# jh-jeong/ContraD

Hardware: AMD Instinct MI355X
Metric: discriminator-step images/sec (ContraD, SimCLR aug) (higher is better)
Workload: dtype f32; 1 GPU; SNDCGAN + ContraD D-step, CIFAR-10 32x32, global batch 512, simclr aug, nonsat loss, Adam(2e-4,(0.5,0.999)), random-init weights; global_batch=512, per_gpu_batch=512, parallelism=dp1, losses_finite=True, launch=hipGraph replay, rccl_ranks=1

## Files before the change

### contrad_amd/csrc/igemm.hip

```cpp
#include "common.h"
#include <stdlib.h>
#include <string.h>
#include <algorithm>
#include <utility>
#include "../../include/contrad_hip.h"

namespace {

enum { MODE_FWD = 0, MODE_DGRAD = 1, MODE_WGRAD = 2 };
#ifndef IGEMM_BK
#define IGEMM_BK 16
#endif
constexpr int BK = IGEMM_BK;
#ifndef IGEMM_MIN_WAVES
#define IGEMM_MIN_WAVES 4
#endif
constexpr int NTHREADS = 256;

struct IgemmArgs {
  const float* A;
  const float* B;
  float* C;
  const float* bias;
  const float* addend;
  const float* act_ref;
  float* bias_ws;
  contrad_conv_desc d;
  float slope, gain;
  int M, Ncol, Kg;
  int tiles_m, tiles_n;
  int P;
  int ptiles_per_split;
  int ny;
  int cgroup;
  int cbal;
  int cb_reps[4], cb_start[5];
  int dsplits;
  long long slab_elems;
  int px_pixels;
  short win_h0[16], win_w0[16], win_hc[16], win_wc[16];
  int win_tile0[17];
  int nwin;
  unsigned char px_order[256];
  int pixmajor;
  int px_full;
  int st_nt;
};

constexpr long long NT_STORE_BYTES = 256ll << 20;
inline int st_nt_for(long long rows, int ld) {
#if defined(LEAN_ST_NT)
  if (LEAN_ST_NT >= 0) return LEAN_ST_NT;
#endif
  return rows * (long long)ld * (long long)sizeof(float) >= NT_STORE_BYTES ? 1 : 0;
}

__device__ __forceinline__ float4 ld4(const float* p) { return *reinterpret_cast<const float4*>(p); }
__device__ __forceinline__ float4 zero4() { return make_float4(0.f, 0.f, 0.f, 0.f); }

template <int MODE, int BM, int BN, bool VEC>
__global__ __launch_bounds__(NTHREADS, 2) void igemm_kernel(const IgemmArgs p) {
  extern __shared__ __attribute__((aligned(16))) float smem[];
  constexpr bool A_KCONTIG = (MODE != MODE_WGRAD);
  constexpr bool B_KCONTIG = (MODE == MODE_DGRAD);
  constexpr int LDA = BM + (A_KCONTIG ? 1 : 4);
  constexpr int LDB = BN + (B_KCONTIG ? 1 : 4);
  constexpr int A_SZ = BK * LDA, B_SZ = BK * LDB;
  constexpr int PA = BM * BK / 1024, PB = BN * BK / 1024;
  constexpr int KQ = BK / 4;
  constexpr int KROWS = NTHREADS / KQ;
  constexpr int WM = BM / 2, WN = BN / 2, TM = WM / 32, TN = WN / 32;
  constexpr int EPV = VEC ? 1 : 4;

  const contrad_conv_desc& d = p.d;
  const int tid = threadIdx.x;
  const int lane = tid & 63, wave = tid >> 6;
  const int wm = wave >> 1, wn = wave & 1;

  const int b = xcd_remap(blockIdx.x, gridDim.x);
  const int tile_n = b % p.tiles_n, tile_m = b / p.tiles_n;
  const int m0 = tile_m * BM, n0 = tile_n * BN;

  int M = p.M, Ncol = p.Ncol, Kg = p.Kg;
  int ph = 0, pw = 0, Hc = 0, Wc = 0, kh0 = 0, kw0 = 0, nth = 0, ntw = 1, bh = 0, bw = 0;
  if constexpr (MODE == MODE_DGRAD) {
    const int s = d.stride;
    ph = blockIdx.y / s;
    pw = blockIdx.y % s;
    Hc = (d.H - ph + s - 1) / s;
    Wc = (d.W - pw + s - 1) / s;
    kh0 = (ph + d.pad) % s;
    kw0 = (pw + d.pad) % s;
    nth = (kh0 < d.KH) ? (d.KH - kh0 + s - 1) / s : 0;
    ntw = (kw0 < d.KW) ? (d.KW - kw0 + s - 1) / s : 0;
    bh = (ph + d.pad - kh0) / s;
    bw = (pw + d.pad - kw0) / s;
    M = d.N * Hc * Wc;
    Ncol = d.C;
    Kg = nth * ntw * d.K;
    if (ntw == 0) ntw = 1;
    if (m0 >= M) return;
  }
  int p_begin = 0, p_end = 0;
  if constexpr (MODE == MODE_WGRAD) {
    p_begin = blockIdx.y * p.ptiles_per_split * BK;
    p_end = min(p.P, p_begin + p.ptiles_per_split * BK);
  }
  const int T = (MODE == MODE_WGRAD) ? ((p_end > p_begin) ? (p_end - p_begin + BK - 1) / BK : 0)
                                     : (Kg + BK - 1) / BK;

  const int kq = tid % KQ, krow = tid / KQ;
  constexpr int A_RPP = 1024 / BM, B_RPP = 1024 / BN;
  const int a_c4 = tid % (BM / 4), a_r = tid / (BM / 4);
  const int b_c4 = tid % (BN / 4), b_r = tid / (BN / 4);

  int a_n[PA], a_h[PA], a_w[PA];
  bool a_ok[PA];
  int wg_dn = 0, wg_dh = 0, wg_dw = 0;
  int wg_pbase = 0;

  if constexpr (MODE == MODE_FWD) {
#pragma unroll
    for (int i = 0; i < PA; ++i) {
      const int m = m0 + krow + KROWS * i;
      a_ok[i] = m < M;
      const int mm = a_ok[i] ? m : 0;
      const int wo = mm % d.Wo, t = mm / d.Wo;
      const int ho = t % d.Ho;
      a_n[i] = t / d.Ho;
      a_h[i] = ho * d.stride - d.pad;
      a_w[i] = wo * d.stride - d.pad;
    }
  } else if constexpr (MODE == MODE_DGRAD) {
#pragma unroll
    for (int i = 0; i < PA; ++i) {
      const int m = m0 + krow + KROWS * i;
      a_ok[i] = m < M;
      const int mm = a_ok[i] ? m : 0;
      const int wq = mm % Wc, t = mm / Wc;
      a_n[i] = t / Hc;
      a_h[i] = t % Hc + bh;
      a_w[i] = wq + bw;
    }
  } else {
    const int hw = d.Ho * d.Wo;
    wg_pbase = p_begin;
    wg_dn = BK / hw;
    const int rem = BK - wg_dn * hw;
    wg_dh = rem / d.Wo;
    wg_dw = rem - wg_dh * d.Wo;
#pragma unroll
    for (int i = 0; i < PA; ++i) {
      const int pp = p_begin + a_r + A_RPP * i;
      const int wo = pp % d.Wo, t = pp / d.Wo;
      a_w[i] = wo;
      a_h[i] = t % d.Ho;
      a_n[i] = t / d.Ho;
      a_ok[i] = true;
    }
  }

  float4 ra[PA], rb[PB];
  unsigned amask = 0, bmask = 0;

  auto fwd_a = [&](int i, int k, bool& ok) -> size_t {
    const int kk = (k < Kg) ? k : 0;
    const int tap = kk / d.C, c = kk - tap * d.C;
    const int kh = tap / d.KW, kw = tap - kh * d.KW;
    const int hi = a_h[i] + kh, wi = a_w[i] + kw;
    ok = (k < Kg) && a_ok[i] && (unsigned)hi < (unsigned)d.H && (unsigned)wi < (unsigned)d.W;
    return ok ? ((size_t)(a_n[i] * d.H + hi) * d.W + wi) * d.ldx + c : 0;
  };
  auto dg_decode = [&](int k, int& th, int& tw, int& co, int& tapflat) {
    const int kk = (k < Kg) ? k : 0;
    const int ti = kk / d.K;
    co = kk - ti * d.K;
    th = ti / ntw;
    tw = ti - th * ntw;
    tapflat = (kh0 + d.stride * th) * d.KW + (kw0 + d.stride * tw);
  };
  auto wg_a = [&](int i, int ic, bool pok, bool& ok) -> size_t {
    const int icc = (ic < Kg) ? ic : 0;
    const int tap = icc / d.C, c = icc - tap * d.C;
    const int kh = tap / d.KW, kw = tap - kh * d.KW;
    const int hi = a_h[i] * d.stride - d.pad + kh, wi = a_w[i] * d.stride - d.pad + kw;
    ok = pok && (ic < Kg) && (unsigned)hi < (unsigned)d.H && (unsigned)wi < (unsigned)d.W;
    return ok ? ((size_t)(a_n[i] * d.H + hi) * d.W + wi) * d.ldx + c : 0;
  };

  auto load_a_generic = [&](int t) {
    const int k0 = t * BK;
    amask = 0;
    if constexpr (MODE == MODE_FWD) {
      const int k = k0 + kq * 4;
#pragma unroll
      for (int i = 0; i < PA; ++i) {
        if constexpr (VEC) {
          bool ok;
          const size_t off = fwd_a(i, k, ok);
          ra[i] = ld4(p.A + off);
// ... 2028 lines not shown
  if (contrad_conv2d_path(d, mode) != 3) return 1.0;
  return mode == MODE_DGRAD ? dgrad_valid_tap_fraction(d) : fwd_valid_tap_fraction(d);
}

extern "C" long long contrad_conv2d_grid_blocks(const contrad_conv_desc* d, int mode, int with_workspace) {
  if (check_desc(d) || mode < 0 || mode > 2) return -22;
  if (mode != MODE_WGRAD && with_workspace && wino44_planned(d, mode)) return wino44_grid(wino44_args(d, mode));
  if (mode != MODE_WGRAD && with_workspace && wino_planned(d, mode)) return wino_grid(wino_args(d, mode));
  if (with_workspace && wino23_planned(d, mode)) return wino23_grid(wino23_args(d));
  if (mode != MODE_WGRAD && with_workspace && wino22_planned(d, mode)) {
    const wino22::Args a = wino22_args(d, mode);
    return 8 * std::min(WINO_CUS / 8, cdiv(a.NTB, 8) * a.NKB * (mode == MODE_DGRAD ? 4 : 1));
  }
  if (mode == MODE_FWD) {
    const FwdPlan p = fwd_plan(d);
    const long long M = (long long)d->N * d->Ho * d->Wo;
    if (fwd_k1_ok(d)) return cdivll(M, 4);
    if (conv_c32_ok(d)) return conv_c32_blocks(d);
    if (p.pixmajor == 1) return (long long)cdiv(d->N, p.bm) * d->Ho * d->Wo * cdiv(d->K, p.bn);
    if (p.pixmajor == 2) return (long long)border_class_tiles(d, MODE_FWD, p.bm) * cdiv(d->K, p.bn);
    return cdivll(M, p.bm) * cdiv(d->K, p.bn) * (with_workspace ? p.splits : 1);
  }
  if (mode == MODE_DGRAD) {
    if (conv_c32_ok(d)) return conv_c32_blocks(d);
    const int s = d->stride;
    const long long Mc = (long long)d->N * cdiv(d->H, s) * cdiv(d->W, s);
    const FwdPlan p = dgrad_plan(d, with_workspace != 0);
    const int tiles_m = p.pixmajor == 2 ? border_class_tiles(d, MODE_DGRAD, p.bm)
                        : p.pixmajor == 1 ? cdiv(d->N, p.bm) * cdiv(d->H, s) * cdiv(d->W, s) : cdiv((int)Mc, p.bm);
    const int tiles_n = cdiv(d->C, p.bn);
    if (p.splits > 1) return (long long)tiles_m * tiles_n * p.splits;
    if (p.balanced && vec_ok(d, MODE_DGRAD) && lean_ok(d, MODE_DGRAD, 0) && p.pixmajor == 0) {
      IgemmArgs a{};
      const long long blocks = dgrad_balance(d, tiles_m, &a);
      if (blocks > 0) return blocks * tiles_n;
    }
    if (p.pixmajor == 1 && s == 2) return (long long)tiles_m * tiles_n * s * s;
    const int cgroup = (s > 1) ? dgrad_cgroup(tiles_m, tiles_n) : 0;
    const int tm_pad = cgroup > 0 ? cdiv(tiles_m, cgroup) * cgroup : tiles_m;
    return (long long)tm_pad * tiles_n * s * s;
  }
  if (wino_wgrad_planned(d)) { const wino::WArgs a = wino_wgrad_args(d); return (long long)a.CB * a.KB * wino_wgrad_splits(a); }
  if (wino22_wgrad_planned(d)) { const wino22::WArgs a = wino22_wgrad_args(d); return (long long)a.RBN * a.KB * wino22_wgrad_splits(a); }
  if (wgrad_c32_ok(d)) return wgrad_c32_blocks(d);
  int bm, bn, tm, tn, splits, pps;
  wgrad_plan(d, &bm, &bn, &tm, &tn, &splits, &pps);
  return (long long)tm * tn * splits;
}

extern "C" int contrad_conv2d_tile_order(const contrad_conv_desc* d, int mode, unsigned char* out, int capacity) {
  if (check_desc(d) || (mode != MODE_FWD && mode != MODE_DGRAD) || !out || capacity <= 0) return -22;
  int taps[256];
  unsigned char full[256];
  int nt = 0;
  if (mode == MODE_FWD) {
    const FwdPlan p = fwd_plan(d);
    if (p.pixmajor != 1 || !vec_ok(d, MODE_FWD)) return 0;
    for (int ho = 0; ho < d->Ho; ++ho)
      for (int wo = 0; wo < d->Wo; ++wo) {
        int vh = 0, vw = 0;
        for (int kh = 0; kh < d->KH; ++kh) vh += (unsigned)(ho * d->stride - d->pad + kh) < (unsigned)d->H;
        for (int kw = 0; kw < d->KW; ++kw) vw += (unsigned)(wo * d->stride - d->pad + kw) < (unsigned)d->W;
        taps[ho * d->Wo + wo] = vh * vw;
      }
    if (!pixel_order_full(taps, d->Ho * d->Wo, cdiv(d->N, p.bm), cdiv(d->K, p.bn), full, 8)) return 0;
    nt = cdiv(d->N, p.bm) * d->Ho * d->Wo;
  } else {
    const FwdPlan p = dgrad_plan(d, true);
    if (p.pixmajor != 1 || p.splits > 1 || !vec_ok(d, MODE_DGRAD)) return 0;
    if (d->stride == 1) {
      for (int h = 0; h < d->H; ++h)
        for (int w = 0; w < d->W; ++w) {
          int vh = 0, vw = 0;
          for (int kh = 0; kh < d->KH; ++kh) vh += (unsigned)(h + d->pad - kh) < (unsigned)d->Ho;
          for (int kw = 0; kw < d->KW; ++kw) vw += (unsigned)(w + d->pad - kw) < (unsigned)d->Wo;
          taps[h * d->W + w] = vh * vw;
        }
      if (!pixel_order_full(taps, d->H * d->W, cdiv(d->N, p.bm), cdiv(d->C, p.bn), full, 8)) return 0;
      nt = cdiv(d->N, p.bm) * d->H * d->W;
    } else {
      const int npix = dgrad_strided_class0_taps(d, taps);
      if (!npix || !dgrad_strided_full_ok(d, p.bm, p.bn)) return 0;
      pixel_order_full(taps, npix, cdiv(d->N, p.bm), cdiv(d->C, p.bn), full, 2);
      nt = cdiv(d->N, p.bm) * npix;
    }
  }
  if (nt > capacity) return -22;
  memcpy(out, full, (size_t)nt);
  return nt;
}

extern "C" long long contrad_conv2d_wgrad_workspace_bytes(const contrad_conv_desc* d) {
  if (check_desc(d)) return -22;
  if (wino_wgrad_planned(d)) return wino_wgrad_workspace_bytes(d);
  if (wino22_wgrad_planned(d)) return wino22_wgrad_workspace_bytes(d);
  if (wgrad_c32_ok(d))
    return (long long)wgrad_c32_blocks(d) * ((long long)d->KH * d->KW * d->C + 1) * d->K * (long long)sizeof(float);
  int bm, bn, tm, tn, splits, pps;
  wgrad_plan(d, &bm, &bn, &tm, &tn, &splits, &pps);
  return (long long)splits * ((long long)d->KH * d->KW * d->C + 1) * d->K * (long long)sizeof(float);
}

extern "C" int contrad_conv2d_wgrad(const contrad_conv_desc* d, const float* x, const float* gy,
                                    float* dwp, float* dbias, float* workspace, long long workspace_bytes,
                                    contrad_stream_t stream) {
  int rc = check_desc(d);
  if (rc) return rc;
  CONTRAD_ARG(x && gy && dwp && workspace);
  if (vec_ok(d, MODE_WGRAD)) CONTRAD_ARG(aligned16(x, gy, workspace));
  CONTRAD_ARG(workspace_bytes >= contrad_conv2d_wgrad_workspace_bytes(d));
  if (wino_wgrad_planned(d)) return launch_wino_wgrad(d, x, gy, dwp, dbias, workspace, (hipStream_t)stream);
  if (wino22_wgrad_planned(d)) return launch_wino22_wgrad(d, x, gy, dwp, dbias, workspace, (hipStream_t)stream);
  if (wgrad_c32_ok(d)) {
    const int blocks = wgrad_c32_blocks(d);
    const long long total = (long long)d->KH * d->KW * d->C * d->K;
    float* bias_ws = dbias ? workspace + (size_t)blocks * total : nullptr;
    rc = launch_wgrad_c32(d, x, gy, workspace, bias_ws, (hipStream_t)stream);
    if (rc) return rc;
    int R = 1;
    while (R < 64 && R * 2 <= blocks && (total / 4) * R < 65536) R <<= 1;
    long long rb = ((total / 4) * R + 255) / 256;
    if (rb > 2048) rb = 2048;
    hipLaunchKernelGGL(wgrad_reduce_kernel, dim3((int)rb), dim3(256), 0, (hipStream_t)stream, workspace, dwp,
                       d->KH * d->KW * d->C, d->K, d->ldw, blocks, bias_ws, dbias, R);
    CONTRAD_CHECK_LAUNCH();
    return 0;
  }
  int bm, bn, splits, pps;
  IgemmArgs a{};
  wgrad_plan(d, &bm, &bn, &a.tiles_m, &a.tiles_n, &splits, &pps);
  a.A = x; a.B = gy; a.C = workspace; a.d = *d;
  a.M = d->KH * d->KW * d->C; a.Ncol = d->K; a.Kg = a.M;
  const bool fused_bias = dbias != nullptr && vec_ok(d, MODE_WGRAD);
  CONTRAD_ARG(dbias == nullptr || fused_bias);
  a.bias_ws = fused_bias ? workspace + (size_t)splits * a.M * a.Ncol : nullptr;
  const long long P = (long long)d->N * d->Ho * d->Wo;
  CONTRAD_ARG(P < (1ll << 31) - 4096);
  a.P = (int)P; a.ptiles_per_split = pps;
  a.pixmajor = wgrad_pixmajor_ok(d, bm, pps) ? 1 : 0;
  rc = dispatch<MODE_WGRAD>(a, bm, bn, vec_ok(d, MODE_WGRAD), dim3(a.tiles_m * a.tiles_n, splits),
                            (hipStream_t)stream);
  if (rc) return rc;
  const long long total = (long long)a.M * a.Ncol;
  int R = 1;
  while (R < 64 && R * 2 <= splits && (total / 4) * R < 65536) R <<= 1;
  long long blocks = ((total / 4) * R + 255) / 256;
  if (blocks > 2048) blocks = 2048;
  if (blocks < 1) blocks = 1;
  hipLaunchKernelGGL(wgrad_reduce_kernel, dim3((int)blocks), dim3(256), 0, (hipStream_t)stream, workspace, dwp,
                     a.M, a.Ncol, d->ldw, splits, a.bias_ws, fused_bias ? dbias : nullptr, R);
  CONTRAD_CHECK_LAUNCH();
  return 0;
}
```

### contrad_amd/csrc/igemm_lean.h

```cpp
#pragma once

#ifndef LEAN_DEEP
#define LEAN_DEEP 0
#endif
#ifndef LEAN_LD_NT
#define LEAN_LD_NT 0
#endif
#ifndef LEAN_ST_NT
#define LEAN_ST_NT -1
#endif
#ifndef LEAN_QPAD
#define LEAN_QPAD 8
#endif

constexpr unsigned LEAN_OOB = 0x80000000u;
constexpr unsigned LEAN_RANGE = 0x80000000u;
constexpr unsigned WB_TOP = 2u, WB_BOT = 4u, WB_LEFT = 8u, WB_RIGHT = 16u;

__device__ __forceinline__ float4 bload4(__amdgpu_buffer_rsrc_t r, unsigned voff, unsigned soff) {
  return __builtin_bit_cast(float4, __builtin_amdgcn_raw_buffer_load_b128(r, (int)voff, (int)soff, 0));
}

__device__ __forceinline__ __amdgpu_buffer_rsrc_t lean_rsrc(const float* base, bool on) {
  return __builtin_amdgcn_make_buffer_rsrc(const_cast<float*>(base), 0, on ? (int)LEAN_RANGE : 0, 0x00020000);
}

template <class P> struct lean_par_value { static constexpr int v = 0; };
template <int V> struct lean_par_value<std::integral_constant<int, V>> { static constexpr int v = V; };

__device__ __forceinline__ int pow2_shift(int d) { return (d & (d - 1)) == 0 ? __builtin_ctz(d) : -1; }
__device__ __forceinline__ void divmod_u(int x, int d, int sh, int& q, int& r) {
  if (sh >= 0) { q = x >> sh; r = x & (d - 1); }
  else { q = x / d; r = x - q * d; }
}

template <int MODE, int BM, int BN, bool BAL>
__device__ __forceinline__ void lean_tile(const IgemmArgs& p, float* smem, const int tile_m, const int tile_n, const int by,
                                          const int wc_h0, const int wc_w0, const int wc_hc, const int wc_wc) {
  static_assert(BK == 16, "the lean loop is written for a 16-deep K-tile");
  static_assert(!BAL || MODE == MODE_DGRAD, "balanced order: strided data gradient only");
  const int pl_pixmajor = BAL ? 0 : p.pixmajor, pl_nwin = BAL ? 0 : p.nwin, pl_dsplits = BAL ? 0 : p.dsplits;
  constexpr bool A_Q = (MODE != MODE_WGRAD);
  constexpr bool B_Q = (MODE == MODE_DGRAD);
  constexpr int QSA = BM * 4 + LEAN_QPAD, QSB = BN * 4 + LEAN_QPAD;
  constexpr int LDB = BN < 64 ? 64 : BN;
  constexpr int A_SZ = A_Q ? 4 * QSA : 16 * BM;
  constexpr int B_SZ = B_Q ? 4 * QSB : 16 * LDB;
  constexpr int BUF = A_SZ + B_SZ;
  constexpr int PA = BM / 64, PB = BN < 64 ? 1 : BN / 64;
  constexpr int A_RPP = 1024 / BM, B_RPP = 1024 / BN;
  constexpr bool B_HALF = BN < 64;
  constexpr int WAVES_N = BN < 64 ? 1 : 2, WAVES_M = 4 / WAVES_N;
  constexpr int WM = BM / WAVES_M, WN = BN / WAVES_N, TM = WM / 32, TN = WN / 32;
  static_assert(TM >= 1 && TN >= 1, "tile too small for the wave arrangement");

  const contrad_conv_desc& d = p.d;
  const int tid = threadIdx.x;
  const int lane = tid & 63, wave = tid >> 6;
  const int wm = wave / WAVES_N, wn = wave % WAVES_N;
  const int l31 = lane & 31, lhi = lane >> 5;

  const int m0 = tile_m * BM, n0 = tile_n * BN;

  const int kq = tid & 3, qrow = tid >> 2;
  const int a_c4 = tid % (BM / 4), a_r = tid / (BM / 4);
  const int b_c4 = tid % (BN / 4), b_r = tid / (BN / 4);

  int M = p.M, Ncol = p.Ncol;
  int T = 0;
  unsigned tapmask = 0xFFFFFFFFu;
  unsigned wskip = 0;
  long long px_off = 0;
  int px_pitch = 0, px_rows = 0;
  const float* baseA = p.A;
  const float* baseB = p.B;
  unsigned va[PA], vb[PB];
  unsigned inv[PA];

  int u_tap = 0, u_a = 0, u_b = 0, u_c0 = 0;
  int u_n = 0, u_h = 0, u_w = 0;
  int ph = 0, pw = 0, Hc = 0, Wc = 0, kh0 = 0, kw0 = 0, nth = 0, ntw = 1, bh = 0, bw = 0;
  int gw = 1, gh = 1, gn = 1, n_begin = 0;

  if constexpr (MODE == MODE_FWD) {
    const int t_total = p.Kg / BK, t_begin = by * p.ptiles_per_split;
    T = min(p.ptiles_per_split, t_total - t_begin);
    if (T < 0) T = 0;
    const int ntaps = d.KH * d.KW;
    u_c0 = (t_begin / ntaps) * BK;
    u_tap = t_begin % ntaps;
    u_a = u_tap / d.KW;
    u_b = u_tap - u_a * d.KW;
    const int HoWo = d.Ho * d.Wo;
    if (pl_pixmajor) {
      int ib, pix;
      if (p.px_full) {
        const int e = p.px_order[tile_m];
        ib = e / HoWo; pix = e - ib * HoWo;
      } else {
        ib = tile_m / HoWo; pix = p.px_order[tile_m - ib * HoWo];
      }
      const int ho = pix / d.Wo, wo = pix - ho * d.Wo;
      const int n_first = ib * BM;
      unsigned wmask = 0, valid = 0;
      for (int kw = 0; kw < d.KW; ++kw) wmask |= ((unsigned)(wo * d.stride - d.pad + kw) < (unsigned)d.W ? 1u : 0u) << kw;
      for (int kh = 0; kh < d.KH; ++kh)
        if ((unsigned)(ho * d.stride - d.pad + kh) < (unsigned)d.H) valid |= wmask << (kh * d.KW);
      tapmask = valid ? valid : 0xFFFFFFFFu;
      T = __builtin_popcount(valid) * (d.C / BK);
      u_tap = valid ? __builtin_ctz(valid) : 0;
      u_a = u_tap / d.KW;
      u_b = u_tap - u_a * d.KW;
      u_c0 = 0;
      baseA = p.A + ((long long)n_first * d.H * d.W + (long long)(ho * d.stride - d.pad) * d.W + (wo * d.stride - d.pad)) * d.ldx;
      const int img = d.H * d.W * d.ldx;
#pragma unroll
      for (int i = 0; i < PA; ++i) {
        const int r = qrow + 64 * i;
        va[i] = (unsigned)((r * img + kq * 4) * 4);
        inv[i] = (n_first + r < d.N) ? 0u : 0xFFFFFFFFu;
      }
      px_off = ((long long)n_first * HoWo + pix) * d.ldy;
      px_pitch = HoWo * d.ldy;
      px_rows = min(BM, d.N - n_first);
    }
    const bool win = pl_nwin > 0;
    const int gHo = win ? wc_hc : d.Ho, gWo = win ? wc_wc : d.Wo;
    if (win) {
      M = d.N * gHo * gWo;
      unsigned wmask = 0, valid = 0;
      for (int kw = 0; kw < d.KW; ++kw) wmask |= ((unsigned)(wc_w0 * d.stride - d.pad + kw) < (unsigned)d.W ? 1u : 0u) << kw;
      for (int kh = 0; kh < d.KH; ++kh)
        if ((unsigned)(wc_h0 * d.stride - d.pad + kh) < (unsigned)d.H) valid |= wmask << (kh * d.KW);
      tapmask = valid ? valid : 0xFFFFFFFFu;
      T = __builtin_popcount(valid) * (d.C / BK);
      u_tap = valid ? __builtin_ctz(valid) : 0;
      u_a = u_tap / d.KW;
      u_b = u_tap - u_a * d.KW;
      u_c0 = 0;
      if (m0 >= M) return;
    }
    const int sh_w = pow2_shift(gWo), sh_h = pow2_shift(gHo);
    const int n_first = (sh_w >= 0 && sh_h >= 0) ? (m0 >> (sh_w + sh_h)) : m0 / (gHo * gWo);
    if (!pl_pixmajor) baseA = p.A + ((long long)n_first * d.H * d.W - (d.pad * d.W + d.pad)) * d.ldx;
#pragma unroll
    for (int i = 0; i < PA; ++i) {
      if (pl_pixmajor) break;
      const int m = m0 + qrow + 64 * i;
      const bool ok = m < M;
      const int mm = ok ? m : m0;
      int wo, t, ho, n;
      divmod_u(mm, gWo, sh_w, t, wo);
      divmod_u(t, gHo, sh_h, n, ho);
      ho += wc_h0; wo += wc_w0;
      va[i] = (unsigned)(((((n - n_first) * d.H + ho * d.stride) * d.W + wo * d.stride) * d.ldx + kq * 4) * 4);
      unsigned wmask = 0, valid = 0;
      for (int kw = 0; kw < d.KW; ++kw) wmask |= ((unsigned)(wo * d.stride - d.pad + kw) < (unsigned)d.W ? 1u : 0u) << kw;
      for (int kh = 0; kh < d.KH; ++kh)
        if ((unsigned)(ho * d.stride - d.pad + kh) < (unsigned)d.H) valid |= wmask << (kh * d.KW);
      inv[i] = ok ? ~valid : 0xFFFFFFFFu;
    }
#pragma unroll
    for (int i = 0; i < PB; ++i) {
      const int col = n0 + b_c4 * 4;
      vb[i] = (col < Ncol && b_r + B_RPP * i < BK) ? (unsigned)((((b_r + B_RPP * i) * d.ldw) + col) * 4) : LEAN_OOB;
    }
  } else if constexpr (MODE == MODE_DGRAD) {
    const int s = d.stride;
    const int cls = (pl_dsplits > 1) ? 0 : by;
    ph = cls / s;
    pw = cls % s;
    Hc = (d.H - ph + s - 1) / s;
    Wc = (d.W - pw + s - 1) / s;
    kh0 = (ph + d.pad) % s;
    kw0 = (pw + d.pad) % s;
    nth = (kh0 < d.KH) ? (d.KH - kh0 + s - 1) / s : 0;
    ntw = (kw0 < d.KW) ? (d.KW - kw0 + s - 1) / s : 0;
    bh = (ph + d.pad - kh0) / s;
    bw = (pw + d.pad - kw0) / s;
    M = d.N * Hc * Wc;
    Ncol = d.C;
    T = nth * ntw * d.K / BK;
    if (pl_dsplits > 1) {
      const int t_begin = by * p.ptiles_per_split, ntaps = nth * ntw;
      T = min(p.ptiles_per_split, T - t_begin);
      if (T < 0) T = 0;
      u_c0 = (t_begin / ntaps) * BK;
      u_tap = t_begin % ntaps;
      u_a = u_tap / ntw;
      u_b = u_tap - u_a * ntw;
    }
    if (ntw == 0) ntw = 1;
    if (pl_nwin > 0) {
      Hc = wc_hc; Wc = wc_wc;
      M = d.N * Hc * Wc;
      const int ah0 = wc_h0 + bh, aw0 = wc_w0 + bw;
      unsigned wmask = 0, valid = 0;
      for (int tw = 0; tw < ntw; ++tw) wmask |= ((unsigned)(aw0 - tw) < (unsigned)d.Wo ? 1u : 0u) << tw;
      for (int th = 0; th < nth; ++th)
        if ((unsigned)(ah0 - th) < (unsigned)d.Ho) valid |= wmask << (th * ntw);
      tapmask = valid ? valid : 0xFFFFFFFFu;
      T = __builtin_popcount(valid) * (d.K / BK);
      u_tap = valid ? __builtin_ctz(valid) : 0;
      u_a = u_tap / ntw;
      u_b = u_tap - u_a * ntw;
      u_c0 = 0;
    }
    const int HcWc = Hc * Wc;
    if (pl_pixmajor) {
      int ib, cpix;
      if (p.px_full) {
        const int e = p.px_order[tile_m];
        ib = e / p.px_pixels; cpix = e - ib * p.px_pixels;
      } else {
        ib = tile_m / p.px_pixels; cpix = p.px_order[tile_m - ib * p.px_pixels];
      }
      if (cpix >= HcWc) return;
      int hq = cpix / Wc, wq = cpix - hq * Wc;
      if (p.px_full == 2) {
        if (ph) hq = Hc - 1 - hq;
        if (pw) wq = Wc - 1 - wq;
      }
      const int ah = hq + bh, aw = wq + bw;
      const int n_first = ib * BM;
      unsigned wmask = 0, valid = 0;
      for (int tw = 0; tw < ntw; ++tw) wmask |= ((unsigned)(aw - tw) < (unsigned)d.Wo ? 1u : 0u) << tw;
      for (int th = 0; th < nth; ++th)
        if ((unsigned)(ah - th) < (unsigned)d.Ho) valid |= wmask << (th * ntw);
      tapmask = valid ? valid : 0xFFFFFFFFu;
      T = __builtin_popcount(valid) * (d.K / BK);
      u_tap = valid ? __builtin_ctz(valid) : 0;
      u_a = u_tap / ntw;
      u_b = u_tap - u_a * ntw;
      u_c0 = 0;
      M = d.N;
      baseA = p.A + ((long long)n_first * d.Ho * d.Wo + (long long)(ah - (nth - 1)) * d.Wo + (aw - (ntw - 1))) * d.ldy;
      const int img = d.Ho * d.Wo * d.ldy;
#pragma unroll
      for (int i = 0; i < PA; ++i) {
        const int r = qrow + 64 * i;
        va[i] = (unsigned)((r * img + kq * 4) * 4);
        inv[i] = (n_first + r < d.N) ? 0u : 0xFFFFFFFFu;
      }
      px_off = ((long long)n_first * d.H * d.W + (long long)(hq * s + ph) * d.W + (wq * s + pw)) * d.ldx;
      px_pitch = d.H * d.W * d.ldx;
      px_rows = min(BM, d.N - n_first);
    }
    if (!pl_pixmajor && m0 >= M) return;
    const int sh_w = pow2_shift(Wc), sh_h = pow2_shift(Hc);
    const int n_first = (sh_w >= 0 && sh_h >= 0) ? (m0 >> (sh_w + sh_h)) : m0 / HcWc;
    if (!pl_pixmajor) baseA = p.A + ((long long)n_first * d.Ho * d.Wo - ((nth - 1) * d.Wo + (ntw - 1))) * d.ldy;
#pragma unroll
    for (int i = 0; i < PA; ++i) {
      if (pl_pixmajor) break;
      const int m = m0 + qrow + 64 * i;
      const bool ok = m < M;
      const int mm = ok ? m : m0;
      int wq, t, n, hq;
      divmod_u(mm, Wc, sh_w, t, wq);
      divmod_u(t, Hc, sh_h, n, hq);
      hq += wc_h0; wq += wc_w0;
      const int ah = hq + bh, aw = wq + bw;
      va[i] = (unsigned)(((((n - n_first) * d.Ho + ah) * d.Wo + aw) * d.ldy + kq * 4) * 4);
      unsigned wmask = 0, valid = 0;
      for (int tw = 0; tw < ntw; ++tw) wmask |= ((unsigned)(aw - tw) < (unsigned)d.Wo ? 1u : 0u) << tw;
      for (int th = 0; th < nth; ++th)
        if ((unsigned)(ah - th) < (unsigned)d.Ho) valid |= wmask << (th * ntw);
      inv[i] = ok ? ~valid : 0xFFFFFFFFu;
    }
#pragma unroll
    for (int i = 0; i < PB; ++i) {
      const int c = n0 + qrow + 64 * i;
      vb[i] = (c < Ncol && qrow + 64 * i < BN) ? (unsigned)((c * d.ldw + kq * 4) * 4) : LEAN_OOB;
    }
  } else {
    const int tiles_total = p.P / BK;
    const int t_begin = by * p.ptiles_per_split;
    T = min(p.ptiles_per_split, tiles_total - t_begin);
    if (T < 0) T = 0;
    gw = min(d.Wo, 16);
    gh = min(d.Ho, 16 / gw);
    if (pl_pixmajor) { gw = 1; gh = 1; }
    gn = 16 / (gw * gh);
    const int tpr = d.Wo / gw, tpi = tpr * (d.Ho / gh);
    u_w = (t_begin % tpr) * gw;
    u_h = ((t_begin / tpr) % (d.Ho / gh)) * gh;
    u_n = (t_begin / tpi) * gn;
    n_begin = u_n;
    baseA = p.A + ((long long)n_begin * d.H * d.W - (d.pad * d.W + d.pad)) * d.ldx;
    baseB = pl_pixmajor ? p.B + (long long)n_begin * d.Ho * d.Wo * d.ldy : p.B + (long long)t_begin * BK * d.ldy;
    if (pl_pixmajor) {
      const int tap0 = m0 / d.C;
      const int kh = tap0 / d.KW, kw = tap0 - kh * d.KW;
      const int chh = kh - d.pad, cww = kw - d.pad;
      const int hb = (d.Ho - 1) * d.stride, wb = (d.Wo - 1) * d.stride;
      wskip = ((unsigned)chh < (unsigned)d.H ? 0u : WB_TOP) | ((unsigned)(hb + chh) < (unsigned)d.H ? 0u : WB_BOT) |
              ((unsigned)cww < (unsigned)d.W ? 0u : WB_LEFT) | ((unsigned)(wb + cww) < (unsigned)d.W ? 0u : WB_RIGHT);
      if (p.bias_ws != nullptr && tile_m == 0) wskip = 0;
      int hh = u_h, ww = u_w, cnt = 0, first = -1;
      for (int q = 0; q < T; ++q) {
        const unsigned e = (hh == 0 ? WB_TOP : 0u) | (hh == d.Ho - 1 ? WB_BOT : 0u) | (ww == 0 ? WB_LEFT : 0u) | (ww == d.Wo - 1 ? WB_RIGHT : 0u);
        if (!(wskip & e)) { ++cnt; if (first < 0) first = q; }
        if (++ww == d.Wo) { ww = 0; if (++hh == d.Ho) hh = 0; }
      }
      T = cnt;
      if (cnt == 0) wskip = 0;
      for (int q = 0; q < first; ++q) {
        u_w += 1;
        if (u_w == d.Wo) { u_w = 0; u_h += 1; if (u_h == d.Ho) { u_h = 0; u_n += gn; } }
      }
    }
    const int ic = m0 + a_c4 * 4;
    const bool colok = ic < p.Kg;
    const int icc = colok ? ic : 0;
    const int tap = icc / d.C, c = icc - tap * d.C;
    const int kh = tap / d.KW, kw = tap - kh * d.KW;
#pragma unroll
    for (int i = 0; i < PA; ++i) {
      const int r = a_r + A_RPP * i;
      const int dw = r % gw, dh = (r / gw) % gh, dn = r / (gw * gh);
      const int chh = dh * d.stride - d.pad + kh, cww = dw * d.stride - d.pad + kw;
      const int hb = (d.Ho - gh) * d.stride, wb = (d.Wo - gw) * d.stride;
      inv[i] = ((unsigned)chh < (unsigned)d.H ? 0u : WB_TOP) | ((unsigned)(hb + chh) < (unsigned)d.H ? 0u : WB_BOT) |
               ((unsigned)cww < (unsigned)d.W ? 0u : WB_LEFT) | ((unsigned)(wb + cww) < (unsigned)d.W ? 0u : WB_RIGHT);
      va[i] = colok ? (unsigned)((((dn * d.H + dh * d.stride + kh) * d.W + dw * d.stride + kw) * d.ldx + c) * 4)
                    : LEAN_OOB;
    }
#pragma unroll
    for (int i = 0; i < PB; ++i) {
      const int col = n0 + b_c4 * 4;
      const int rowpitch = pl_pixmajor ? d.Ho * d.Wo * d.ldy : d.ldy;
      vb[i] = (col < Ncol && b_r + B_RPP * i < BK) ? (unsigned)((((b_r + B_RPP * i) * rowpitch) + col) * 4) : LEAN_OOB;
    }
  }

  constexpr bool DEEP = ((LEAN_DEEP & 1) && MODE == MODE_WGRAD && BM * BN <= 128 * 64) ||
                        ((LEAN_DEEP & 2) && MODE != MODE_WGRAD && BM * BN <= 128 * 64);
  constexpr int NSET = DEEP ? 2 : 1;
  float4 ra[NSET][PA], rb[NSET][PB];
  unsigned soffA = 0, soffB = 0;
  unsigned edge = 0;
  auto wgrad_pos_edge = [&]() -> unsigned {
    return (u_h == 0 ? WB_TOP : 0u) | (u_h == d.Ho - gh ? WB_BOT : 0u) | (u_w == 0 ? WB_LEFT : 0u) | (u_w == d.Wo - gw ? WB_RIGHT : 0u);
  };
  unsigned pos_edge = (MODE == MODE_WGRAD) ? wgrad_pos_edge() : 0u;
  unsigned pos_offA = 0, pos_offB = 0, wk_aw = 0, wk_ah = 0, wk_an = 0, wk_b = 0, wk_bh = 0, wk_bn = 0;
  (void)wk_bh;
  if constexpr (MODE == MODE_FWD) {
    pos_offA = (unsigned)(((u_a * d.W + u_b) * d.ldx + u_c0) * 4);
    pos_offB = (unsigned)((u_tap * d.C + u_c0) * d.ldw * 4);
    wk_aw = (unsigned)(d.ldx * 4);
    wk_ah = (unsigned)((d.W - d.KW) * d.ldx * 4);
    wk_an = (unsigned)((BK - d.KH * d.W * d.ldx) * 4);
    wk_b = (unsigned)(d.C * d.ldw * 4);
    wk_bn = (unsigned)((BK - d.KH * d.KW * d.C) * d.ldw * 4);
  } else if constexpr (MODE == MODE_DGRAD) {
    pos_offA = (unsigned)((((nth - 1 - u_a) * d.Wo + (ntw - 1 - u_b)) * d.ldy + u_c0) * 4);
    pos_offB = (unsigned)((((kh0 + d.stride * u_a) * d.KW + (kw0 + d.stride * u_b)) * d.C * d.ldw + u_c0) * 4);
    wk_aw = (unsigned)(-d.ldy * 4);
    wk_ah = (unsigned)((ntw - d.Wo) * d.ldy * 4);
    wk_an = (unsigned)((nth * d.Wo * d.ldy + BK) * 4);
    wk_b = (unsigned)(d.stride * d.C * d.ldw * 4);
    wk_bh = (unsigned)(d.stride * (d.KW - ntw) * d.C * d.ldw * 4);
    wk_bn = (unsigned)((BK - d.stride * nth * d.KW * d.C * d.ldw) * 4);
  }
  if constexpr (MODE == MODE_WGRAD) {
    pos_offA = (unsigned)(((((u_n - n_begin) * d.H + u_h * d.stride) * d.W + u_w * d.stride) * d.ldx) * 4);
    pos_offB = pl_pixmajor ? (unsigned)((((u_n - n_begin) * d.Ho + u_h) * d.Wo + u_w) * d.ldy * 4) : 0u;
    wk_aw = (unsigned)(gw * d.stride * d.ldx * 4);
    wk_ah = (unsigned)((gh * d.stride * d.W - d.Wo * d.stride) * d.ldx * 4);
    wk_an = (unsigned)((gn * d.H - d.Ho * d.stride) * d.W * d.ldx * 4);
    wk_b = (unsigned)((pl_pixmajor ? 1 : BK) * d.ldy * 4);
    wk_bn = pl_pixmajor ? (unsigned)((gn - 1) * d.Ho * d.Wo * d.ldy * 4) : 0u;
  }
  int t_next = 0;
  __amdgpu_buffer_rsrc_t rsA = lean_rsrc(baseA, false), rsB = lean_rsrc(baseB, false);

  auto begin_tile = [&]() {
    const bool on = t_next < T;
    rsA = lean_rsrc(baseA, on);
    rsB = lean_rsrc(baseB, on);
    soffA = pos_offA;
    soffB = pos_offB;
    if constexpr (MODE == MODE_WGRAD) edge = pos_edge;
  };
  auto end_tile = [&]() {
    ++t_next;
    if constexpr (MODE == MODE_FWD) {
      do {
        ++u_tap; ++u_b; pos_offA += wk_aw; pos_offB += wk_b;
        if (u_b == d.KW) {
          u_b = 0; ++u_a; pos_offA += wk_ah;
          if (u_a == d.KH) { u_a = 0; u_tap = 0; pos_offA += wk_an; pos_offB += wk_bn; }
        }
      } while (!((tapmask >> u_tap) & 1u));
    } else if constexpr (MODE == MODE_DGRAD) {
      do {
        ++u_tap; ++u_b; pos_offA += wk_aw; pos_offB += wk_b;
        if (u_b == ntw) {
          u_b = 0; ++u_a; pos_offA += wk_ah; pos_offB += wk_bh;
          if (u_a == nth) { u_a = 0; u_tap = 0; pos_offA += wk_an; pos_offB += wk_bn; }
        }
      } while (!((tapmask >> u_tap) & 1u));
    } else {
      do {
        u_w += gw; pos_offA += wk_aw; pos_offB += wk_b;
        if (u_w == d.Wo) {
          u_w = 0; u_h += gh; pos_offA += wk_ah;
          if (u_h == d.Ho) { u_h = 0; u_n += gn; pos_offA += wk_an; pos_offB += wk_bn; }
        }
        pos_edge = wgrad_pos_edge();
      } while (wskip & pos_edge);
    }
  };
  auto load_a_piece = [&](int set, int i) {
    unsigned v;
    if constexpr (MODE == MODE_WGRAD) {
      v = (inv[i] & edge) ? LEAN_OOB : va[i];
    } else {
      v = va[i] | ((inv[i] >> u_tap) << 31);
    }
    ra[set][i] = bload4(rsA, v, soffA);
  };
  auto load_b_piece = [&](int set, int i) { rb[set][i] = bload4(rsB, vb[i], soffB); };

  int wrA, wrB, rdA[TM], rdB[TN];
  if constexpr (A_Q) {
    wrA = kq * QSA + qrow * 4;
#pragma unroll
    for (int i = 0; i < TM; ++i) rdA[i] = lhi * QSA + (wm * WM + i * 32 + l31) * 4;
  } else {
    wrA = a_r * BM + ((a_c4 * 4) ^ (((a_r >> 2) & 1) * 32));
#pragma unroll
    for (int i = 0; i < TM; ++i) rdA[i] = 4 * lhi * BM + ((wm * WM + i * 32 + l31) ^ (32 * lhi));
  }
  if constexpr (B_Q) {
    wrB = A_SZ + kq * QSB + qrow * 4;
#pragma unroll
    for (int j = 0; j < TN; ++j) rdB[j] = A_SZ + lhi * QSB + (wn * WN + j * 32 + l31) * 4;
  } else {
    wrB = A_SZ + b_r * LDB + ((b_c4 * 4) ^ (((b_r >> 2) & 1) * 32));
#pragma unroll
    for (int j = 0; j < TN; ++j) rdB[j] = A_SZ + 4 * lhi * LDB + ((wn * WN + j * 32 + l31) ^ (32 * lhi));
  }

  float4 colacc = zero4();
  const bool do_bias = (MODE == MODE_WGRAD) && p.bias_ws != nullptr && tile_m == 0;

  auto store_a_piece = [&](int bufoff, int set, int i) {
    float* dst = smem + bufoff + wrA + (A_Q ? i * 256 : i * A_RPP * BM);
    *reinterpret_cast<float4*>(dst) = ra[set][i];
  };
  const bool b_owner = !B_HALF || (B_Q ? qrow < BN : b_r < BK);
  auto store_b_piece = [&](int bufoff, int set, int i) {
    float* dst = smem + bufoff + wrB + (B_Q ? i * 256 : i * B_RPP * LDB);
    if (b_owner) *reinterpret_cast<float4*>(dst) = rb[set][i];
    if constexpr (MODE == MODE_WGRAD) {
      if (do_bias) {
        asm volatile("" ::: "memory");
        colacc.x += rb[set][i].x; colacc.y += rb[set][i].y; colacc.z += rb[set][i].z; colacc.w += rb[set][i].w;
      }
    }
  };

  f32x16 acc[TM][TN];
#pragma unroll
  for (int i = 0; i < TM; ++i)
#pragma unroll
    for (int j = 0; j < TN; ++j)
#pragma unroll
      for (int r = 0; r < 16; ++r) acc[i][j][r] = 0.f;

  if (T > 0) {
    begin_tile();
#pragma unroll
    for (int i = 0; i < PA; ++i) load_a_piece(0, i);
#pragma unroll
    for (int i = 0; i < PB; ++i) load_b_piece(0, i);
    end_tile();
    if constexpr (DEEP) {
      begin_tile();
#pragma unroll
      for (int i = 0; i < PA; ++i) load_a_piece(1, i);
#pragma unroll
      for (int i = 0; i < PB; ++i) load_b_piece(1, i);
      end_tile();
    }
#pragma unroll
    for (int i = 0; i < PA; ++i) store_a_piece(0, 0, i);
#pragma unroll
    for (int i = 0; i < PB; ++i) store_b_piece(0, 0, i);
  }
  __syncthreads();

  constexpr bool RAGGED_SKIP = (MODE == MODE_WGRAD) && BN <= 64;
  const bool wave_on = !RAGGED_SKIP || __builtin_amdgcn_readfirstlane((m0 + wm * WM < M) ? 1 : 0) != 0;

  constexpr int KS = BK / 2;
#ifndef IGEMM_ST_SHIFT
#define IGEMM_ST_SHIFT 1
#endif
  constexpr int A_LD0 = 0, B_LD0 = PA, A_ST0 = KS - PA - PB - IGEMM_ST_SHIFT, B_ST0 = KS - PB - IGEMM_ST_SHIFT;
  static_assert(A_ST0 >= A_LD0 + PA - 1 && B_ST0 >= B_LD0 + PB - 1 && A_ST0 >= 0,
                "a piece must be stored after its own load was issued");
  constexpr bool UNROLL2 = !(BM * BN > 128 * 64 && MODE != MODE_WGRAD);
  static_assert(!DEEP || UNROLL2, "the two-deep prefetch needs the buffer parity at compile time");
  auto k_tile = [&](auto par, auto with_mfma, const int t) {
    const int cur = (int)par * BUF, nxt = BUF - cur;
    (void)t;
    float fa[2][TM][4], fb[2][TN][4];
#if defined(LEAN_ABLATE_FRAGS)
#pragma unroll
    for (int h = 0; h < 2; ++h)
#pragma unroll
      for (int j = 0; j < 4; ++j) {
#pragma unroll
        for (int i = 0; i < TM; ++i) fa[h][i][j] = (float)(t + i + j);
#pragma unroll
        for (int i = 0; i < TN; ++i) fb[h][i][j] = (float)(t - i - j);
      }
#else
#pragma unroll
    for (int h = 0; h < 2; ++h) {
#pragma unroll
      for (int i = 0; i < TM; ++i) {
        if constexpr (A_Q) {
          const float4 q = *reinterpret_cast<const float4*>(smem + cur + rdA[i] + 2 * h * QSA);
          fa[h][i][0] = q.x; fa[h][i][1] = q.y; fa[h][i][2] = q.z; fa[h][i][3] = q.w;
        } else {
#pragma unroll
          for (int j = 0; j < 4; ++j) fa[h][i][j] = smem[cur + rdA[i] + (8 * h + j) * BM];
        }
      }
#pragma unroll
      for (int i = 0; i < TN; ++i) {
        if constexpr (B_Q) {
          const float4 q = *reinterpret_cast<const float4*>(smem + cur + rdB[i] + 2 * h * QSB);
          fb[h][i][0] = q.x; fb[h][i][1] = q.y; fb[h][i][2] = q.z; fb[h][i][3] = q.w;
        } else {
#pragma unroll
          for (int j = 0; j < 4; ++j) fb[h][i][j] = smem[cur + rdB[i] + (8 * h + j) * LDB];
        }
      }
    }
#endif
    __builtin_amdgcn_sched_barrier(0);
#pragma unroll
    for (int ks = 0; ks < KS; ++ks) {
      const int h = ks >> 2, j = ks & 3;
#if !defined(LEAN_ABLATE_LOADS)
      constexpr int LSET = DEEP ? lean_par_value<decltype(par)>::v : 0, SSET = DEEP ? 1 - lean_par_value<decltype(par)>::v : 0;
      if (ks == A_LD0) begin_tile();
      if (ks >= A_LD0 && ks < A_LD0 + PA) load_a_piece(LSET, ks - A_LD0);
      if (ks >= B_LD0 && ks < B_LD0 + PB) load_b_piece(LSET, ks - B_LD0);
      if (ks == B_LD0 + PB - 1) end_tile();
#endif
      __builtin_amdgcn_sched_barrier(0);
      if constexpr (decltype(with_mfma)::value) {
#pragma unroll
        for (int i = 0; i < TM; ++i)
#pragma unroll
          for (int jj = 0; jj < TN; ++jj)
            acc[i][jj] = __builtin_amdgcn_mfma_f32_32x32x2f32(fa[h][i][j], fb[h][jj][j], acc[i][jj], 0, 0, 0);
      }
      __builtin_amdgcn_sched_barrier(0);
// ... 114 lines not shown
          }
        }
      }
    };
    if (st_nt && !(MODE == MODE_DGRAD && pl_dsplits > 1)) store_rows(std::true_type{}); else store_rows(std::false_type{});
  } else {
    const bool slab = (MODE == MODE_WGRAD) || p.ny > 1;
    const bool pxm = (MODE == MODE_FWD) && pl_pixmajor;
    const int pitch = pxm ? px_pitch : (slab ? Ncol : d.ldy);
    const size_t out_off = pxm ? (size_t)px_off : (slab ? (size_t)by * M * Ncol : (size_t)0) + (size_t)m0 * pitch;
    float* outp = p.C + out_off;
    const int rows_here = pxm ? px_rows : min(BM, M - m0);
    const __amdgpu_buffer_rsrc_t rsC = __builtin_amdgcn_make_buffer_rsrc(outp, 0, rows_here * pitch * 4, 0x00020000);
    const int wave_row = __builtin_amdgcn_readfirstlane(wm * WM);
    const float g1 = p.gain, g0 = p.gain * p.slope;
    const bool has_add = (MODE == MODE_FWD) && !slab && p.addend != nullptr;
    const __amdgpu_buffer_rsrc_t rsD = __builtin_amdgcn_make_buffer_rsrc(
        const_cast<float*>(has_add ? p.addend + out_off : outp), 0, has_add ? rows_here * pitch * 4 : 0, 0x00020000);
    unsigned lanepart[TN];
    float bj[TN];
#pragma unroll
    for (int j = 0; j < TN; ++j) {
      lanepart[j] = colpart[j] + (unsigned)(4 * lhi * pitch) * 4u;
      const int c = n0 + wn * WN + j * 32 + l31;
      bj[j] = (MODE == MODE_FWD && !slab && p.bias && c < Ncol) ? p.bias[c] : 0.f;
    }
    if constexpr (MODE == MODE_FWD) {
      constexpr int EPI_F = (BM * BN > 128 * 64) ? 4 : EPI_G;
      auto store_fwd = [&](auto nt_c) {
      constexpr int ST_AUX = decltype(nt_c)::value ? 2 : 0;
      constexpr int LD_AUX = (LEAN_LD_NT && decltype(nt_c)::value) ? 2 : 0;
#pragma unroll
      for (int i = 0; i < TM; ++i)
#pragma unroll
        for (int r0 = 0; r0 < 16; r0 += EPI_F) {
          unsigned rowpart[EPI_F];
#pragma unroll
          for (int q = 0; q < EPI_F; ++q) {
            const int r = r0 + q;
            rowpart[q] = (unsigned)((wave_row + i * 32 + (r & 3) + 8 * (r >> 2)) * pitch) * 4u;
          }
          float rv[EPI_F][TN];
          if (has_add) {
#pragma unroll
            for (int q = 0; q < EPI_F; ++q)
#pragma unroll
              for (int j = 0; j < TN; ++j)
                rv[q][j] = __builtin_bit_cast(float, __builtin_amdgcn_raw_buffer_load_b32(rsD, (int)(lanepart[j] + rowpart[q]), 0, LD_AUX));
          }
#pragma unroll
          for (int q = 0; q < EPI_F; ++q)
#pragma unroll
            for (int j = 0; j < TN; ++j) {
              float v = acc[i][j][r0 + q];
              if (!slab) {
                v += bj[j];
                v *= (v > 0.f) ? g1 : g0;
                if (has_add) v += rv[q][j];
              }
              __builtin_amdgcn_raw_buffer_store_b32(__builtin_bit_cast(unsigned, v), rsC, (int)(lanepart[j] + rowpart[q]), 0, ST_AUX);
            }
        }
      };
      if (st_nt && !slab) store_fwd(std::true_type{}); else store_fwd(std::false_type{});
    } else {
#pragma unroll
      for (int i = 0; i < TM; ++i)
#pragma unroll
        for (int r = 0; r < 16; ++r) {
          const unsigned rowpart = (unsigned)((wave_row + i * 32 + (r & 3) + 8 * (r >> 2)) * pitch) * 4u;
#pragma unroll
          for (int j = 0; j < TN; ++j) {
            const float v = acc[i][j][r];
            __builtin_amdgcn_raw_buffer_store_b32(__builtin_bit_cast(unsigned, v), rsC, (int)(lanepart[j] + rowpart), 0, 0);
          }
        }
    }
    if constexpr (MODE == MODE_WGRAD) {
      if (do_bias) {
        float* red = smem;
        *reinterpret_cast<float4*>(red + b_r * BN + b_c4 * 4) = colacc;
        __syncthreads();
        if (tid < BN) {
          float sum = 0.f;
#pragma unroll
          for (int r = 0; r < B_RPP; ++r) sum += red[r * BN + tid];
          const int c = n0 + tid;
          if (c < Ncol) p.bias_ws[(size_t)by * Ncol + c] = sum;
        }
      }
    }
  }
}

template <int MODE, int BM, int BN, bool BAL = false>
__global__ __launch_bounds__(NTHREADS, IGEMM_MIN_WAVES) void igemm_lean_kernel(const IgemmArgs p) {
  extern __shared__ __attribute__((aligned(16))) float smem[];
  const int lin = xcd_remap(blockIdx.x, gridDim.x);
  int by, tile_n, tile_m;
  int nrep = 1;
  int wc_h0 = 0, wc_w0 = 0, wc_hc = 0, wc_wc = 0;
  if constexpr (MODE == MODE_WGRAD) {
    const int tiles = p.tiles_m * p.tiles_n;
    by = lin / tiles;
    const int b = lin - by * tiles;
    tile_n = b % p.tiles_n; tile_m = b / p.tiles_n;
  } else if constexpr (BAL) {
    const int per_group = p.cb_start[4] * p.tiles_n;
    const int g = lin / per_group, r = lin - g * per_group;
    const int blk = r / p.tiles_n;
    tile_n = r - blk * p.tiles_n;
    by = (blk >= p.cb_start[1]) + (blk >= p.cb_start[2]) + (blk >= p.cb_start[3]);
    nrep = p.cb_reps[by];
    tile_m = g * p.cbal + (blk - p.cb_start[by]) * nrep;
    if (tile_m >= p.tiles_m) return;
  } else if (MODE == MODE_DGRAD && p.cgroup > 0) {
    const int per_group = p.cgroup * p.ny * p.tiles_n;
    const int g = lin / per_group, r = lin - g * per_group;
    by = r / (p.cgroup * p.tiles_n);
    const int q = r - by * (p.cgroup * p.tiles_n);
    tile_m = g * p.cgroup + q / p.tiles_n;
    tile_n = q % p.tiles_n;
    if (tile_m >= p.tiles_m) return;
  } else if (MODE != MODE_WGRAD && p.nwin > 0) {
    const int xcd = blockIdx.x & 7, kb = blockIdx.x >> 3;
    tile_n = kb % p.tiles_n;
    int km = kb / p.tiles_n, c = 0;
    tile_m = -1;
    for (; c < p.nwin; ++c) {
      const int n_c = p.win_tile0[c + 1] - p.win_tile0[c];
      const int lo = (xcd * n_c) >> 3, hi = ((xcd + 1) * n_c) >> 3;
      if (km < hi - lo) { tile_m = lo + km; break; }
      km -= hi - lo;
    }
    if (tile_m < 0) return;
    by = 0;
    wc_h0 = p.win_h0[c]; wc_w0 = p.win_w0[c]; wc_hc = p.win_hc[c]; wc_wc = p.win_wc[c];
  } else {
    tile_n = lin % p.tiles_n;
    const int r = lin / p.tiles_n;
    by = r % p.ny; tile_m = r / p.ny;
  }
  if constexpr (BAL) {
    for (int rep = 0; rep < nrep; ++rep) {
      lean_tile<MODE, BM, BN, true>(p, smem, tile_m + rep, tile_n, by, 0, 0, 0, 0);
      if (rep + 1 < nrep) __syncthreads();
    }
  } else {
    lean_tile<MODE, BM, BN, false>(p, smem, tile_m, tile_n, by, wc_h0, wc_w0, wc_hc, wc_wc);
  }
}

template <int MODE, int BM, int BN>
constexpr size_t lean_smem_bytes() {
  const int a = (MODE != MODE_WGRAD) ? 4 * (BM * 4 + LEAN_QPAD) : 16 * BM;
  const int b = (MODE == MODE_DGRAD) ? 4 * (BN * 4 + LEAN_QPAD) : 16 * (BN < 64 ? 64 : BN);
  size_t main_loop = 2 * (size_t)(a + b) * sizeof(float);
  size_t epi = (size_t)BM * sizeof(long long);
  return main_loop > epi ? main_loop : epi;
}
```

### contrad_amd/engine.py

```python
import os

import torch
import torch.distributed as dist

from . import ops as _ops
from .hostio import THROTTLE


FORCE_DIST = False


def dist_on():
    return dist.is_available() and dist.is_initialized() and (dist.get_world_size() > 1 or FORCE_DIST)


_dist_on = dist_on


class GradAllReducer(object):

    SMALL = 1 << 18

    def __init__(self, params):
        self.params = [p for p in params]
# ... 89 lines not shown
    if world > 1:
        opt_D.step(grad_scale=1.0 / world)
    else:
        opt_D.step()
    THROTTLE.end()
    return d_loss, aux


def r1_loss(D, images, augment_fn):
    from . import autograd_ops as A
    images_aug = augment_fn(images).detach()
    images_aug.requires_grad = True
    d_real = D(images_aug)
    with A.input_grad_only():
        grad_real, = torch.autograd.grad(outputs=d_real.sum(), inputs=images_aug, create_graph=True, retain_graph=True)
    return A.SumSqMeanFn.apply(grad_real)


def _sg2_fakes(G, N, style_mix):
    if hasattr(G, 'draw_inputs'):
        return G(**G.draw_inputs(N, style_mix))
    return G(G.sample_latent(N), style_mix=style_mix)


def d_step_stylegan2(P, G, D, opt_D, options, images, step, reducer=None, style_mix=0.9):
    THROTTLE.begin()
    with torch.no_grad():
        gen_images = _sg2_fakes(G, images.size(0), style_mix)
    d_loss, aux = P.train_fn["D"](P, D, options, images, gen_images)
    loss = d_loss + aux['penalty']
    if (step % P.d_reg_every == 0) and P.lbd_r1 > 0:
        r1 = r1_loss(D, images, P.augment_fn)
        loss = torch.add(loss, r1, alpha=(0.5 * P.lbd_r1) * P.d_reg_every)
        aux['r1'] = r1
    opt_D.zero_grad()
    loss.backward()
    world = reducer() if reducer is not None else 1
    opt_D.step(grad_scale=1.0 / world) if world > 1 else opt_D.step()
    THROTTLE.end()
    return d_loss, aux


_MERGED_CALLS = os.environ.get('CONTRAD_DEV_MERGED', '1') != '0'


def loss_D_fn_separate(P, D, options, images, gen_images):
    from .training.gan.contrad import _ContraDContrastive, _GanDLoss
    N = images.size(0)
    if _MERGED_CALLS and hasattr(D, 'call_merged') and getattr(P.augment_fn, 'supports_out', False):
        both = torch.empty((3 * N,) + tuple(images.shape[1:]), device=images.device, dtype=torch.float32)
        P.augment_fn(gen_images.detach(), out=both[2 * N:])
        P.augment_fn(torch.cat([images, images], dim=0), out=both[:2 * N])
        d_all, aux = D.call_merged(both, [2 * N, N], sg_linear=True, projection=True, projection2=True)
        proj, proj2 = aux['projection'], aux['projection2']
    else:
        aug_f = P.augment_fn(gen_images.detach())
        aug_r = P.augment_fn(torch.cat([images, images], dim=0))
        if hasattr(D, 'call_batches'):
            (d_gen, aux_g), (d_real2, aux_r) = D.call_batches([aug_f, aug_r], sg_linear=True, projection=True,
                                                              projection2=True)
        else:
            d_gen, aux_g = D(aug_f, sg_linear=True, projection=True, projection2=True)
            d_real2, aux_r = D(aug_r, sg_linear=True, projection=True, projection2=True)
        proj = torch.cat([aux_r['projection'], aux_g['projection']], dim=0)
        proj2 = torch.cat([aux_r['projection2'], aux_g['projection2']], dim=0)
        d_all = torch.cat([d_real2, d_gen], dim=0)
    simclr, sup = _ContraDContrastive.apply(proj, proj2, N, P.temp, bool(P.distributed))
    gan, d_real_m, d_gen_m = _GanDLoss.apply(d_all, N, options['loss'])
    return simclr + P.lbd_a * sup, {'penalty': gan, 'd_real': d_real_m, 'd_gen': d_gen_m}


def d_step_stylegan2_contrad(P, G, D, opt_D, options, images, step, reducer=None, style_mix=0.9):
    N = images.size(0)
    THROTTLE.begin()
    with torch.no_grad():
        gen_images = _sg2_fakes(G, N, style_mix)
    d_loss, aux = loss_D_fn_separate(P, D, options, images, gen_images)
    loss = d_loss + aux['penalty']
    if (step % P.d_reg_every == 0) and P.lbd_r1 > 0:
        r1 = r1_loss(D, images, P.augment_fn)
        loss = torch.add(loss, r1, alpha=(0.5 * P.lbd_r1) * P.d_reg_every)
        aux['r1'] = r1
    opt_D.zero_grad()
    loss.backward()
    world = reducer() if reducer is not None else 1
    opt_D.step(grad_scale=1.0 / world) if world > 1 else opt_D.step()
    THROTTLE.end()
    return d_loss, aux


def _quiesce_before_capture(*modules):
    for m in modules:
        if hasattr(m, 'drop_pack_cache'):
            m.drop_pack_cache()
    torch.cuda.synchronize()
    if dist.is_available() and dist.is_initialized():
        import time
        time.sleep(1.0)
        torch.cuda.synchronize()
        return 'thread_local'
    return 'global'


class GraphedDStep(object):

    def __init__(self, P, G, D, opt_D, options, images, warmup=3):
        from .augment import SimCLRAugment
        from . import ops
        self.P, self.G, self.D, self.opt, self.options = P, G, D, opt_D, options
        self.aug = P.augment_fn
        if not isinstance(self.aug, SimCLRAugment) or self.aug.p_blur is not None:
            raise NotImplementedError('GraphedDStep: the simclr pipeline')
        self.dist = dist_on()
        self.reducer = None
        if self.dist and getattr(D, '_grad_comm', None) is None:
            self.reducer = GradAllReducer(D.parameters())
        self.images = images.clone()
        N = images.size(0)
        dev = images.device
        self.N = N
        for _ in range(warmup if len(opt_D.state) else max(warmup, 1)):
            d_step(P, G, D, opt_D, options, images, self.reducer)
        self.z = torch.zeros(N, G.nz, device=dev)
        self.params = torch.zeros(3 * N, ops.AUG_NPARAM, device=dev)
        self.hyper = torch.ones(3, device=dev)
        torch.cuda.synchronize()
        G.invalidate_cache()
        self.graph = torch.cuda.CUDAGraph()
        self._scratch = {}
        mode = _quiesce_before_capture(self.D)
        if _ops.SEQUENCE is not None:
            _ops.SEQUENCE.append('capture')
        with _ops.private_workspace(self._scratch), torch.cuda.graph(self.graph, capture_error_mode=mode):
            self.d_loss, self.aux = self._body()
        G.invalidate_cache()
        torch.cuda.synchronize()

    def load_images(self, images):
        self.images.copy_(images)

    def _refresh_inputs(self):
        from .hostio import upload_into
        G, N = self.G, self.N
        z = torch.empty(N, G.nz).uniform_(-1, 1)
        Pm, cf, _ = self.aug.sample(3 * N, self.images.shape[2], self.images.shape[3])
        Pm[:, 15] = float(cf)
        upload_into(z, self.z)
        upload_into(Pm, self.params)
        world = dist.get_world_size() if self.dist else 1
        upload_into(torch.tensor([self.opt.hyper_values(1.0 / world)], dtype=torch.float32), self.hyper.view(1, 3))

    def _body(self):
        from . import ops
        from .training.gan.contrad import _ContraDContrastive, _GanDLoss
        P, G, D, N = self.P, self.G, self.D, self.N
        with torch.no_grad():
            gen = G(self.z)
            cat = torch.cat([self.images, self.images, gen], dim=0)
            aug = ops.simclr_augment(cat, self.params, -1, self.aug.r_c is not None)
        d_all, aux = D(aug, sg_linear=True, projection=True, projection2=True)
        simclr, sup = _ContraDContrastive.apply(aux['projection'], aux['projection2'], N, P.temp,
                                                bool(P.distributed) and self.dist)
        gan, d_real, d_gen = _GanDLoss.apply(d_all, N, self.options['loss'])
        d_loss = simclr + P.lbd_a * sup
        self.opt.zero_grad(set_to_none=True)
        (d_loss + gan).backward()
        if self.reducer is not None:
            self.reducer()
        self.opt.step_captured(self.hyper)
        return d_loss.detach(), {'penalty': gan.detach(), 'd_real': d_real.detach(), 'd_gen': d_gen.detach()}

    def __call__(self):
        THROTTLE.begin()
        self._refresh_inputs()
        self.graph.replay()
        THROTTLE.end()
        return self.d_loss, self.aux


class _StaticAugment(object):

    def __init__(self, aug, sizes, H, W, device):
        from . import ops
        self.aug, self.sizes, self.H, self.W, self.dev = aug, list(sizes), H, W, device
        self.blocks = [torch.zeros(n, ops.AUG_NPARAM, device=device) for n in self.sizes]
        self.radius = int((H // 10) / 2) if aug.p_blur is not None else 0
        self.taps = [torch.zeros(2 * self.radius + 1, device=device) for _ in self.sizes] if self.radius > 0 else None
        self.k = 0

    def refresh(self):
        from .hostio import upload
        for i, n in enumerate(self.sizes):
            Pm, _cf, sigma = self.aug.sample(n, self.H, self.W)
            self.blocks[i].copy_(upload(Pm, self.dev))
            if self.taps is not None:
                _r, g = self.aug.blur_kernel(self.H, sigma)
                self.taps[i].copy_(upload(g.view(1, -1), self.dev).view(-1))

    supports_out = True

    def __call__(self, x, out=None):
        from . import ops
        i, self.k = self.k, self.k + 1
        if x.shape[0] != self.sizes[i]:
            raise RuntimeError('captured step: augmentation call %d saw %d images, planned %d' % (i, x.shape[0], self.sizes[i]))
        if x.requires_grad and torch.is_grad_enabled():
            from .augment import _SimCLRFn
            if out is not None:
                raise RuntimeError('augmentation: out= is a forward-only option')
            return _SimCLRFn.apply(x.contiguous().float(), self.blocks[i], -1, self.aug.r_c is not None,
                                   (self.radius, self.taps[i]) if self.taps is not None else None,
                                   self.aug.cutout_length if self.aug.p_cutout is not None else None)
        res = ops.simclr_augment(x.detach().contiguous().float(), self.blocks[i], -1, self.aug.r_c is not None,
                                 out=None if self.taps is not None else out)
        if self.taps is not None:
            res = ops.gaussian_blur_masked(res, self.blocks[i], self.taps[i], self.radius, out=out)
        if self.aug.p_cutout is not None:
            ops.cutout_masked_(res, self.blocks[i], self.aug.cutout_length)
        return res


class _StaticSG2Inputs(object):

    def __init__(self, G, N, device, style_mix):
        self.G, self.N, self.dev, self.style_mix = G, N, device, style_mix
        self.flat = torch.zeros(sum(G.input_sizes(N)), device=device)
        self.mix_layer = torch.zeros(N, device=device)
        self.mixing = G.training and style_mix > 0
        z, z_mix, noise = G.input_views(self.flat, N)
        self.kw = dict(input=z, style_mix=style_mix, noise=noise)
        if self.mixing:
            self.kw['_mix'] = (z_mix, self.mix_layer)

    def refresh(self):
        from .hostio import upload
        G, N = self.G, self.N
        self.flat.normal_()
        if self.mixing:
            nomix = torch.rand(N) >= self.style_mix
            mix_layer = torch.randint(G.n_latent, (N,)).masked_fill(nomix, G.n_latent)
            self.mix_layer.copy_(upload(mix_layer.float().view(-1, 1), self.dev).view(-1))

    def forward(self):
        return self.G(**self.kw)


class GraphedSG2DStep(object):

    def __init__(self, P, G, D, opt_D, options, images, contrad_script, style_mix=0.9, warmup=2):
        import argparse
        self.dist = dist_on()
        self.reducer = None
        if self.dist:
            rest = D.overlap_rest() if getattr(D, '_pack_comm', None) is not None else None
            self.reducer = GradAllReducer(rest if rest is not None else D.parameters())
        self.P, self.G, self.D, self.opt, self.options, self.images = P, G, D, opt_D, options, images.clone()
        self.contrad_script, self.style_mix = contrad_script, style_mix
        self.eager = d_step_stylegan2_contrad if contrad_script else d_step_stylegan2
        N, dev = images.size(0), images.device
        self.N = N
        self.r1_in_graph = P.lbd_r1 > 0 and P.d_reg_every == 1
        for s in range(1, (warmup if len(opt_D.state) else max(warmup, 1)) + 1):
            self.eager(P, G, D, opt_D, options, images, s if P.d_reg_every == 1 else 1, self.reducer, style_mix)
        H, W = images.shape[2], images.shape[3]
        sizes = ([N, 2 * N] if contrad_script else [3 * N]) + ([N] if self.r1_in_graph else [])
        self.saug = _StaticAugment(P.augment_fn, sizes, H, W, dev)
        self.Pg = argparse.Namespace(**vars(P))
        self.Pg.augment_fn = self.saug
        self.gin = _StaticSG2Inputs(G, N, dev, style_mix)
        self.hyper = torch.ones(3, device=dev)
        torch.cuda.synchronize()
        G.invalidate_cache()
        self.graph = torch.cuda.CUDAGraph()
        self._scratch = {}
        mode = _quiesce_before_capture(self.D)
        if _ops.SEQUENCE is not None:
            _ops.SEQUENCE.append('capture')
        with _ops.private_workspace(self._scratch), torch.cuda.graph(self.graph, capture_error_mode=mode):
            self.d_loss, self.aux = self._body()
        G.invalidate_cache()
        torch.cuda.synchronize()

    def load_images(self, images):
        self.images.copy_(images)

    def _refresh(self):
        from .hostio import upload
        dev = self.images.device
        self.gin.refresh()
        self.saug.refresh()
        world = dist.get_world_size() if self.dist else 1
        self.hyper.copy_(upload(torch.tensor([self.opt.hyper_values(1.0 / world)], dtype=torch.float32), dev).view(3))

    def _body(self):
        P, G, D = self.Pg, self.G, self.D
        self.saug.k = 0
        with torch.no_grad():
            gen = self.gin.forward()
        if self.contrad_script:
            d_loss, aux = loss_D_fn_separate(P, D, self.options, self.images, gen)
        else:
            d_loss, aux = P.train_fn["D"](P, D, self.options, self.images, gen)
        loss = d_loss + aux['penalty']
        if self.r1_in_graph:
            r1 = r1_loss(D, self.images, self.saug)
            loss = torch.add(loss, r1, alpha=(0.5 * P.lbd_r1) * P.d_reg_every)
            aux['r1'] = r1
        self.opt.zero_grad(set_to_none=True)
        loss.backward()
        if self.reducer is not None:
            self.reducer()
        self.opt.step_captured(self.hyper)
        return d_loss.detach(), {k: v.detach() for k, v in aux.items()}
# ... 117 lines not shown
```

### contrad_amd/models/gan/base.py

```python
import math

import torch
import torch.nn as nn
import torch.nn.functional as F


class SNParams(nn.Module):

    def __init__(self, weight_shape, init_std=0.02):
        super().__init__()
        out = weight_shape[0]
        inn = int(math.prod(weight_shape[1:]))
        self.bias = nn.Parameter(torch.zeros(out))
        self.weight_orig = nn.Parameter(torch.empty(*weight_shape))
        self.register_buffer('weight_u', torch.empty(out))
        self.register_buffer('weight_v', torch.empty(inn))
        self.init_std = init_std
        self.reset_parameters()

    def reset_parameters(self):
        with torch.no_grad():
            self.weight_orig.normal_(0.0, self.init_std)
            self.bias.zero_()
            self.weight_u.copy_(F.normalize(torch.randn(self.weight_u.shape), dim=0, eps=1e-12))
            self.weight_v.copy_(F.normalize(torch.randn(self.weight_v.shape), dim=0, eps=1e-12))

    def extra_repr(self):
        return 'weight=%s (spectral norm)' % (tuple(self.weight_orig.shape),)


class PlainParams(nn.Module):

    def __init__(self, weight_shape, bias=True):
        super().__init__()
        self.weight = nn.Parameter(torch.empty(*weight_shape))
        self.bias = nn.Parameter(torch.zeros(weight_shape[0])) if bias else None
        self.reset_parameters()

    def reset_parameters(self):
        fan_in = int(math.prod(self.weight.shape[1:]))
        bound = 1.0 / math.sqrt(fan_in)
        with torch.no_grad():
            self.weight.uniform_(-bound, bound)
            if self.bias is not None:
                self.bias.uniform_(-bound, bound)


class _Act(nn.Module):

    def __init__(self, slope):
        super().__init__()
        self.slope = slope

    def extra_repr(self):
        return 'LeakyReLU(%g), fused into the producing kernel' % self.slope


class TinyHead(nn.Module):

    def __init__(self, n_features, d_hidden, spectral):
        super().__init__()
        mk = SNParams if spectral else PlainParams
        self.l1 = mk((d_hidden, n_features))
        self.l2 = mk((1, d_hidden))


class _LinHeadFn(torch.autograd.Function):

    @staticmethod
    def forward(ctx, feats, weight, bias):
        from ... import ops
        ctx.save_for_backward(feats, weight)
        ctx.has_bias = bias is not None
        return ops.linhead_fwd(feats, weight, bias)[0]

    @staticmethod
    def backward(ctx, g):
        from ... import ops
        feats, weight = ctx.saved_tensors
        g = g.contiguous()
        gw = gb = gf = None
        if ctx.needs_input_grad[1] or (ctx.has_bias and ctx.needs_input_grad[2]):
            gw, gb = torch.empty_like(weight), g.new_empty(weight.shape[0])
            ops.linhead_wgrad_sgd(feats, g, grad_weight=gw, grad_bias=gb)
        if ctx.needs_input_grad[0]:
            gf = g @ weight
        return gf, gw, (gb if ctx.has_bias else None)


class LinearWrapper(nn.Linear):

    def __init__(self, in_features, out_features, bias=True):
        super().__init__(in_features, out_features, bias)

    def forward(self, inputs, y=None):
        if not inputs.is_cuda:
            return F.linear(inputs, self.weight, self.bias)
        lead = inputs.shape[:-1]
        flat = inputs.reshape(-1, inputs.shape[-1]).float()
        if flat.stride(-1) != 1:
            flat = flat.contiguous()
        return _LinHeadFn.apply(flat, self.weight, self.bias).view(*lead, self.out_features)


def make_projection(n_features, d_hidden, d_project, spectral):
    mk = SNParams if spectral else PlainParams
    return nn.Sequential(mk((d_hidden, n_features)), _Act(0.1), mk((d_project, d_hidden)))


class BaseDiscriminator(nn.Module):

    d_penul = None

    def __setattr__(self, name, value):
        if name == 'linear' and isinstance(value, LinearWrapper) and isinstance(self._modules.get('linear'), TinyHead):
            self.__dict__['_stock_head'] = self._modules['linear']
        super().__setattr__(name, value)

    def _head(self):
        lin = self._modules['linear']
        return self.__dict__['_stock_head'] if isinstance(lin, LinearWrapper) else lin

    def _apply(self, fn, *args, **kwargs):
        out = super()._apply(fn, *args, **kwargs)
        if '_stock_head' in self.__dict__:
            self.__dict__['_stock_head']._apply(fn, *args, **kwargs)
        return out

    def _run(self, inputs, sg_linear, finetuning, want_features):
        raise NotImplementedError

    def forward(self, inputs, y=None, penultimate=False, projection=False, projection2=False,
                finetuning=False, sg_linear=False):
        if y is not None:
            raise NotImplementedError('class-conditional heads (n_classes > 1) are not used by get_architecture')
        lin = self._modules.get('linear')
        replaced = isinstance(lin, LinearWrapper)
        want_features = penultimate or replaced
        if getattr(self, '_lazy_projections', False):
            output, project, project2, features = self._run(inputs, sg_linear, finetuning, want_features,
                                                            want_proj=(projection or projection2))
        else:
            output, project, project2, features = self._run(inputs, sg_linear, finetuning, want_features)
        if replaced:
            output = lin(features.detach() if (sg_linear or finetuning) else features)
        aux = {}
        if penultimate:
            aux['penultimate'] = features
        if projection:
            aux['projection'] = project
        if projection2:
            aux['projection2'] = project2
        if aux:
            return output, aux
        return output

    def reset_parameters(self, root=None):
        root = self if root is None else root
        for m in root.modules():
            if isinstance(m, (SNParams, PlainParams)):
                m.reset_parameters()
```

### contrad_amd/models/gan/sndcgan.py

```python
import torch
import torch.nn as nn
import torch.distributed as dist

from ... import ops
from ...hostio import upload
from ... import autograd_ops as A
from .base import BaseDiscriminator, SNParams, TinyHead, _Act, make_projection

_D_CONVS = [(3, 64, 3, 1, 1), (64, 128, 4, 2, 1), (128, 128, 3, 1, 1), (128, 256, 4, 2, 1),
            (256, 256, 3, 1, 1), (256, 512, 4, 2, 1), (512, 512, 3, 1, 1)]
_SLOPE = 0.1


def _flat_views(total_sizes, device):
    offs, tot = [], 0
    for n in total_sizes:
        offs.append(tot)
        tot += ops.round_up(n, 4)
    buf = torch.empty(max(tot, 4), device=device, dtype=torch.float32)
    return buf, [buf[o:o + n] for o, n in zip(offs, total_sizes)]


class _DPlan(object):

    def __init__(self, D, device):
        self.hb = D.s_hb
        self.wb = D.s_wb
        dh, dp = D.d_hidden, D.d_project
        self.dh, self.dp = dh, dp
        convs = [D.main[2 * i] for i in range(7)]
        heads1 = [D._head().l1, D.projection[0], D.projection2[0]]
        heads2 = [D._head().l2, D.projection[2], D.projection2[2]]
        self.layers = convs + heads1 + heads2
        T_head = self.hb * self.wb
        self.specs = []
        for m in convs:
            self.specs.append(ops.SnSpec(m.weight_orig, m.weight_u, m.weight_v))
        for m in heads1:
            self.specs.append(ops.SnSpec(m.weight_orig, m.weight_u, m.weight_v, view_kct=(dh, 512, T_head)))
        for m in heads2:
            self.specs.append(ops.SnSpec(m.weight_orig, m.weight_u, m.weight_v))
        sizes = [s.T * s.C * s.K for s in self.specs[:7]]
        sizes.append(T_head * 512 * 3 * dh)
        sizes += [dh * 4, dh * dp, dh * dp]
        self.pack_sizes = sizes
        self.feat = T_head * 512

    def alloc_packed(self, device):
        buf, v = _flat_views(self.pack_sizes, device)
        dh, dp = self.dh, self.dp
        wps, ldws = [], []
        for i, s in enumerate(self.specs[:7]):
            wps.append(v[i].view(s.T * s.C, s.K)); ldws.append(s.K)
        merged = v[7].view(self.feat, 3 * dh)
        for j in range(3):
            wps.append(merged[:, j * dh:(j + 1) * dh]); ldws.append(3 * dh)
        wps.append(v[8].view(dh, 4)); ldws.append(4)
        wps.append(v[9].view(dh, dp)); ldws.append(dp)
        wps.append(v[10].view(dh, dp)); ldws.append(dp)
        return buf, wps, ldws, merged


class _DFunction(torch.autograd.Function):
    @staticmethod
    def forward(ctx, D, images, sg_linear, want_features, trunk_grad, *params):
        dev = images.device
        plan = _DPlan(D, dev)
        specs = plan.specs
        n = len(specs)
        training = D.training
        B = images.shape[0]
        dh, dp = plan.dh, plan.dp

        wbuf, wps, ldws, merged = plan.alloc_packed(dev)
        offs, scr_n = ops.sn_scratch_floats(specs)
        snap_sizes = []
        for s in specs:
            snap_sizes += [s.K, s.C * s.T]
        snapbuf, snaps = _flat_views(snap_sizes, dev)
        u_snaps, v_snaps = snaps[0::2], snaps[1::2]
        scratch = torch.empty(scr_n, device=dev, dtype=torch.float32)
        sigma = torch.empty(n, device=dev, dtype=torch.float32)
        if trunk_grad:
            ops.sn_weight_prep(specs, wps, ldws, training, scratch, offs, sigma, u_snaps, v_snaps)
        else:
            ops.sn_weight_prep(specs[:7], wps[:7], ldws[:7], False, scratch, offs[:7], sigma, u_snaps[:7], v_snaps[:7])
            ops.sn_weight_prep(specs[7:], wps[7:], ldws[7:], training, scratch, offs[7:], sigma[7:], u_snaps[7:],
                               v_snaps[7:])

        filters = None
        if ops.FILTER_PREP:
            reqs, hw = [], (images.shape[2], images.shape[3])
            for i in range(1, 7):
                ci, co, k, s, p = _D_CONVS[i]
                d = ops.fwd_desc((B, hw[0], hw[1], ci), wps[i], co, k, k, s, p)
                reqs.append((0, d, wps[i]))
                if trunk_grad:
                    reqs.append((1, d, wps[i]))
                hw = (d.Ho, d.Wo)
            filters = ops.filter_prep(reqs, dev)

        biases = [m.bias for m in plan.layers]
        acts = []
        x = ops.rgb_conv_fwd(images, wps[0], biases[0], 64, 3, 2.0, -1.0, _SLOPE, 1.0)
        acts.append(x)
        for i in range(1, 7):
            ci, co, k, s, p = _D_CONVS[i]
            x = ops.conv2d_fwd(x, wps[i], biases[i], co, k, k, s, p, _SLOPE, 1.0, filters=filters)
            acts.append(x)
        bias_cat = torch.cat([biases[7], biases[8], biases[9]])
        hidden = ops.conv2d_fwd(x.view(B, 1, 1, plan.feat), merged, bias_cat, 3 * dh, 1, 1, 1, 0, _SLOPE, 1.0)
        logits = ops.conv2d_fwd(hidden[..., 0:dh], wps[10], biases[10], 1, 1, 1, 1, 0).view(B, 1)
        proj = ops.conv2d_fwd(hidden[..., dh:2 * dh], wps[11], biases[11], dp, 1, 1, 1, 0).view(B, dp)
        proj2 = ops.conv2d_fwd(hidden[..., 2 * dh:3 * dh], wps[12], biases[12], dp, 1, 1, 1, 0).view(B, dp)

        if getattr(D, '_record_activations', False):
            D._last_activations = (acts, hidden)
        ctx.plan, ctx.D = plan, D
        ctx.images, ctx.acts, ctx.hidden = images, acts, hidden
        ctx.wps, ctx.ldws, ctx.merged, ctx.wbuf, ctx.filters = wps, ldws, merged, wbuf, filters
        ctx.sigma, ctx.u_snaps, ctx.v_snaps, ctx.snapbuf = sigma, u_snaps, v_snaps, snapbuf
        ctx.sg_linear, ctx.trunk_grad = sg_linear, trunk_grad
        ctx.param_shapes = [tuple(p.shape) for p in params]
        if want_features:
            feats = x.permute(0, 3, 1, 2).reshape(B, -1)
        else:
            feats = logits.new_empty(0)
            ctx.mark_non_differentiable(feats)
        return logits, proj, proj2, feats

    @staticmethod
    def backward(ctx, g_logits, g_proj, g_proj2, g_feats):
        plan, D = ctx.plan, ctx.D
        specs, wps, ldws = plan.specs, ctx.wps, ctx.ldws
        acts, hidden, images = ctx.acts, ctx.hidden, ctx.images
        dev = images.device
        B = images.shape[0]
        dh, dp = plan.dh, plan.dp
        n = len(specs)
        need_params = any(ctx.needs_input_grad[5:])
        need_images = ctx.needs_input_grad[1]
        a6 = acts[6]
        comm = getattr(D, '_grad_comm', None)

        def exchange(t):
            if comm is not None:
                comm.reduce_async(t)

        def _c(g, shape):
            if g is None:
                return torch.zeros(shape, device=dev, dtype=torch.float32)
            return g.contiguous()

        g_logits = _c(g_logits, (B, 1)).view(B, 1, 1, 1)
        g_proj = _c(g_proj, (B, dp)).view(B, 1, 1, dp)
        g_proj2 = _c(g_proj2, (B, dp)).view(B, 1, 1, dp)

        if need_params:
            gbuf, gv = _flat_views(plan.pack_sizes, dev)
            gwps = []
            for i, s in enumerate(specs[:7]):
                gwps.append(gv[i].view(s.T * s.C, s.K))
            gmerged = gv[7].view(plan.feat, 3 * dh)
            for j in range(3):
                gwps.append(gmerged[:, j * dh:(j + 1) * dh])
            gwps += [gv[8].view(dh, 4), gv[9].view(dh, dp), gv[10].view(dh, dp)]
            bsizes = [m.bias.numel() for m in plan.layers]
            bbuf, gbias = _flat_views(bsizes, dev)

        g_hidden = torch.empty((B, 1, 1, 3 * dh), device=dev, dtype=torch.float32)
        outs = [(g_logits, 10, 0), (g_proj, 11, 1), (g_proj2, 12, 2)]
        for g, li, j in outs:
            hs = hidden[..., j * dh:(j + 1) * dh]
            ops.conv2d_dgrad(g, wps[li], (B, 1, 1, dh), 1, 1, 1, 0, act_ref=hs, slope=_SLOPE, gain=1.0,
                             out=g_hidden[..., j * dh:(j + 1) * dh])
            if need_params:
                if g.shape[3] % 4 == 0:
                    ops.conv2d_wgrad(hs, g, 1, 1, 1, 0, out=gwps[li], dbias=gbias[li])
                else:
                    ops.conv2d_wgrad(hs, g, 1, 1, 1, 0, out=gwps[li])
                    ops.colstats(ops.as_rows(g), out=gbias[li].view(1, -1))
                exchange(gwps[li])
        if need_params:
            o7 = gbias[7].storage_offset()
            adjacent = all(gbias[7 + j].storage_offset() == o7 + j * dh for j in range(3))
            gb_hidden = bbuf[o7:o7 + 3 * dh] if adjacent else torch.empty(3 * dh, device=dev, dtype=torch.float32)
            ops.conv2d_wgrad(a6.view(B, 1, 1, plan.feat), g_hidden, 1, 1, 1, 0, out=gmerged, dbias=gb_hidden)
            exchange(gmerged)
            if not adjacent:
                for j in range(3):
                    gbias[7 + j].copy_(gb_hidden[j * dh:(j + 1) * dh])
        g = None
        if ctx.trunk_grad:
            lo = dh if ctx.sg_linear else 0
            fused = g_feats is None or g_feats.numel() == 0
            g = ops.conv2d_dgrad(g_hidden[..., lo:], ctx.merged[:, lo:], (B, 1, 1, plan.feat), 1, 1, 1, 0,
                                 act_ref=a6.view(B, 1, 1, plan.feat) if fused else None, slope=_SLOPE,
                                 gain=1.0).view(a6.shape)
            if not fused:
                g = g + g_feats.reshape(B, 512, plan.hb, plan.wb).permute(0, 2, 3, 1)
                g = (g * torch.where(a6 > 0, 1.0, _SLOPE)).contiguous()
            for i in range(6, 0, -1):
                ci, co, k, s, p = _D_CONVS[i]
                if need_params:
                    ops.conv2d_wgrad(acts[i - 1], g, k, k, s, p, out=gwps[i], dbias=gbias[i])
                    exchange(gwps[i])
                g = ops.conv2d_dgrad(g, wps[i], tuple(acts[i - 1].shape), k, k, s, p, act_ref=acts[i - 1],
                                     slope=_SLOPE, gain=1.0, filters=ctx.filters)
            if need_params:
                ops.rgb_conv_wgrad(images, g, 3, 2.0, -1.0, gwps[0], gbias[0])
                exchange(gwps[0])
        d_images = None
        if need_images and g is not None:
            d_images = ops.rgb_conv_dgrad(g, wps[0], None, 3, 3, act=0, out_scale=2.0, out_shift=0.0)

        grads = [None] * (2 * n)
        if need_params:
            if g is None:
                for i in range(7):
                    gwps[i].zero_(); gbias[i].zero_()
                    exchange(gwps[i])
            if comm is not None:
                exchange(bbuf)
                comm.wait()
            wsizes = [s.K * s.C * s.T for s in specs]
            gwbuf, gws = _flat_views(wsizes, dev)
            offs, scr_n = ops.sn_scratch_floats(specs)
            scratch = torch.empty(scr_n, device=dev, dtype=torch.float32)
            ops.sn_weight_grad(specs, wps, ldws, gwps, gws, scratch, offs, ctx.sigma, ctx.u_snaps, ctx.v_snaps)
            for i in range(n):
                grads[2 * i] = gws[i].view(ctx.param_shapes[2 * i])
                grads[2 * i + 1] = gbias[i]
        return (None, d_images, None, None, None) + tuple(grads)


class D_SNDCGAN(BaseDiscriminator):

    def __init__(self, image_size, ndf=64, n_classes=1, normalize=False, disable_sn=False, mlp_linear=True,
                 d_hidden=512, d_project=128):
        super().__init__()
        if ndf != 64 or n_classes != 1 or normalize or disable_sn or not mlp_linear:
            raise NotImplementedError('only the configuration built by get_architecture("sndcgan") is implemented')
        s_h, s_w, nc = image_size
        if nc != 3 or s_h % 8 or s_w % 8:
            raise NotImplementedError('RGB images with sides divisible by 8')
        self.image_size = image_size
        self.s_hb, self.s_wb = s_h // 8, s_w // 8
        self.n_features = 512 * self.s_hb * self.s_wb
        self.d_penul = self.n_features
        self.n_classes, self.d_hidden, self.d_project = n_classes, d_hidden, d_project

        self.linear = TinyHead(self.n_features, d_hidden, spectral=True)
        self.projection = make_projection(self.n_features, d_hidden, d_project, spectral=True)
        self.projection2 = make_projection(self.n_features, d_hidden, d_project, spectral=True)
        layers = []
        for (ci, co, k, s, p) in _D_CONVS:
            layers += [SNParams((co, ci, k, k)), _Act(_SLOPE)]
        self.main = nn.Sequential(*layers)

    def enable_grad_overlap(self, comm):
        self._grad_comm = comm

    def _ordered_params(self):
        out = []
        for m in ([self.main[2 * i] for i in range(7)] +
                  [self._head().l1, self.projection[0], self.projection2[0],
                   self._head().l2, self.projection[2], self.projection2[2]]):
            out += [m.weight_orig, m.bias]
        return out

    def _run(self, inputs, sg_linear, finetuning, want_features):
        if not inputs.is_cuda:
            raise RuntimeError('contrad_amd.D_SNDCGAN runs on the MI355X HIP path only (no CPU fallback)')
        if finetuning:
            inputs = inputs.detach()
        images = inputs.contiguous().float()
        logits, proj, proj2, feats = _DFunction.apply(self, images, bool(sg_linear), bool(want_features),
                                                      not finetuning, *self._ordered_params())
        return logits, proj, proj2, (feats if want_features else None)

    def penultimate(self, inputs):
        return self._run(inputs, False, False, True)[3]


class BNParams(nn.Module):

    def __init__(self, c, eps=1e-5, momentum=0.1):
        super().__init__()
        self.eps, self.momentum = eps, momentum
        self.weight = nn.Parameter(torch.ones(c))
        self.bias = nn.Parameter(torch.zeros(c))
        self.register_buffer('running_mean', torch.zeros(c))
        self.register_buffer('running_var', torch.ones(c))
        self.register_buffer('num_batches_tracked', torch.tensor(0, dtype=torch.long))


def _sync_on(flag):
    from ...engine import dist_on
    return flag and dist_on()


class _BNReLUFn(torch.autograd.Function):

    @staticmethod
    def forward(ctx, x2d, gamma, beta, bn, conv_bias, sync):
        x2d = x2d.contiguous()
        stats = ops.colstats(x2d, with_sq=True)
        count = float(x2d.shape[0])
        if _sync_on(sync):
            dist.all_reduce(stats)
            count *= dist.get_world_size()
        if bn.training:
            ops.bn_running_update(stats, count, conv_bias, bn.momentum, bn.running_mean, bn.running_var,
                                  bn.num_batches_tracked)
        y = torch.empty_like(x2d)
        ops.bn_relu_apply(x2d, y, stats, count, gamma, beta, bn.eps)
        ctx.save_for_backward(x2d, stats, gamma, beta)
        ctx.cfg = (count, bn.eps, sync)
        ctx.cb_shape = tuple(conv_bias.shape) if (conv_bias is not None and conv_bias.requires_grad) else None
        return y

    @staticmethod
    def backward(ctx, dy):
        x2d, stats, gamma, beta = ctx.saved_tensors
        count, eps, sync = ctx.cfg
        red = (lambda t: dist.all_reduce(t)) if _sync_on(sync) else None
        dx, dgamma, dbeta = ops.bn_relu_bwd(dy.contiguous(), x2d, stats, count, gamma, beta, eps, red)
        dcb = torch.zeros(ctx.cb_shape, device=dy.device, dtype=dy.dtype) if ctx.cb_shape is not None else None
        return dx, dgamma, dbeta, None, dcb, None


class _WB(nn.Module):
    def __init__(self, wshape, nbias):
        super().__init__()
        self.weight = nn.Parameter(torch.empty(*wshape).normal_(0.0, 0.02))
        self.bias = nn.Parameter(torch.zeros(nbias))


class G_SNDCGAN(nn.Module):

    _CONVT = [(512, 256, 4, 2, 1), (256, 128, 4, 2, 1), (128, 64, 4, 2, 1), (64, 3, 3, 1, 1)]

    def __init__(self, image_size, ngf=64, nz=128):
        super().__init__()
        if ngf != 64:
            raise NotImplementedError('ngf = 64')
        s_h, s_w, nc = image_size
        self.image_size, self.ngf, self.nz = image_size, ngf, nz
        self.s_hb, self.s_wb = s_h // 8, s_w // 8
        f = ngf * 8 * self.s_hb * self.s_wb
        self.linear = _WB((f, nz), f)
        self.norm_init = BNParams(f)
        layers = []
        for j, (ci, co, k, s, p) in enumerate(self._CONVT):
            layers.append(_WB((ci, co, k, k), co))
            if j < 3:
                layers += [BNParams(co), _Act(0.0)]
            else:
                layers.append(_Act(1.0))
        self.main = nn.Sequential(*layers)
        self.sync_bn = True
        self._packed = None
        self._packed_key = None
        self._packed_filters = {}

    def sample_latent(self, n_samples):
        _device = next(self.parameters()).device
        return upload(torch.empty(n_samples, self.nz).uniform_(-1, 1), _device)

    def invalidate_cache(self):
        self._packed, self._packed_key, self._packed_filters = None, None, {}

    def _weights(self):
        ws = [self.linear.weight] + [self.main[3 * j].weight for j in range(4)]
        key = tuple((w.data_ptr(), w._version) for w in ws)
        if self._packed_key != key:
            dev = ws[0].device
            specs = [ops.SnSpec(w, fixed_scale=1.0) for w in ws]
            sizes = [s.K * s.C * s.T for s in specs]
            buf, v = _flat_views(sizes, dev)
            wps = [v[i].view(s.T * s.C, s.K) for i, s in enumerate(specs)]
            ldws = [s.K for s in specs]
            offs, scr_n = ops.sn_scratch_floats(specs)
            scratch = torch.empty(scr_n, device=dev, dtype=torch.float32)
            sigma = torch.empty(len(specs), device=dev, dtype=torch.float32)
            ops.sn_weight_prep(specs, wps, ldws, False, scratch, offs, sigma)
            self._packed, self._packed_key, self._packed_buf = wps, key, buf
            self._packed_filters = {}
        return self._packed

    def _filters(self, N):
        if not ops.FILTER_PREP:
            return None
        pf = self._packed_filters.get(N)
        if pf is None:
            reqs, H, W = [], self.s_hb, self.s_wb
            for j in range(3):
                ci, co, k, s, p = self._CONVT[j]
                H, W = 2 * H, 2 * W
                reqs.append((1, ops.dgrad_desc((N, H, W, co), self._packed[1 + j], ci, k, k, s, p), self._packed[1 + j]))
            pf = self._packed_filters[N] = ops.filter_prep(reqs, self._packed[0].device)
        return pf

    def _bn(self, x2d, bn, conv_bias, out2d, perm_hw=1):
        if not self.training:
            mean = bn.running_mean if conv_bias is None else bn.running_mean - conv_bias
            stats = torch.stack([mean, bn.running_var + mean * mean]).contiguous()
            ops.bn_relu_apply(x2d, out2d, stats, 1.0, bn.weight, bn.bias, bn.eps, perm_hw)
            return
        count = float(x2d.shape[0])
        if ops.BN_FUSED and not _sync_on(self.sync_bn):
            stats = ops.bn_batch_stats(x2d, conv_bias, bn.momentum, bn.running_mean, bn.running_var, bn.num_batches_tracked)
            ops.bn_relu_apply(x2d, out2d, stats, count, bn.weight, bn.bias, bn.eps, perm_hw)
            return
        stats = ops.colstats(x2d, with_sq=True)
        if _sync_on(self.sync_bn):
            dist.all_reduce(stats)
            count *= dist.get_world_size()
        if self.training:
            ops.bn_running_update(stats, count, conv_bias, bn.momentum, bn.running_mean, bn.running_var,
                                  bn.num_batches_tracked)
        ops.bn_relu_apply(x2d, out2d, stats, count, bn.weight, bn.bias, bn.eps, perm_hw)

    def _forward_with_grad(self, z):
        N = z.shape[0]
        hb, wb = self.s_hb, self.s_wb
        f = 512 * hb * wb
        entries = [(f, self.nz, 1, 1.0, 0, 0)]
        groups = [(self.nz, f)]
        ws = [self.linear.weight]
        for j, (ci, co, k, s, p) in enumerate(self._CONVT):
# ... 44 lines not shown
```

### contrad_amd/ops.py

```python
import ctypes
import os

import torch

from ._lib import ConvDesc, ContrastProblem, FilterBatch, FilterJob, FILTER_MAX_JOBS, L2normProblem, lib


def _p(t):
    return ctypes.c_void_p(t.data_ptr()) if t is not None else ctypes.c_void_p(0)


_raw_stream = getattr(torch._C, '_cuda_getCurrentRawStream', None)


def _stream_handle():
    if _raw_stream is not None:
        return _raw_stream(torch.cuda.current_device())
    return torch.cuda.current_stream().cuda_stream


def _stream():
    return ctypes.c_void_p(_stream_handle())


def _chk(t, name):
    if t is None:
        return
    if not t.is_cuda or t.dtype != torch.float32:
        raise RuntimeError('contrad_hip: %s must be a CUDA float32 tensor (got %s, %s)' % (name, t.device, t.dtype))
    if t.dim() > 0 and t.numel() > 0 and t.stride(-1) != 1:
        raise RuntimeError('contrad_hip: %s must be contiguous in its last dimension' % name)


def _ld(t):
    if t.dim() == 4:
        N, H, W, C = t.shape
        ld = t.stride(2) if W > 1 else (t.stride(1) if H > 1 else (t.stride(0) if N > 1 else C))
        if (W > 1 and t.stride(1) != W * ld) or (H * W > 1 and N > 1 and t.stride(0) != H * W * ld):
            raise RuntimeError('contrad_hip: NHWC view must be dense over (N,H,W)')
        return ld
    if t.dim() == 2:
        return t.stride(0) if t.size(0) > 1 else max(t.size(1), t.stride(0))
    raise RuntimeError('contrad_hip: expected a 2-D or 4-D tensor')


def round_up(x, m):
    return (x + m - 1) // m * m


def out_size(h, k, stride, pad):
    return (h + 2 * pad - k) // stride + 1


PROFILE = None
PROFILE_ONLY = None
SEQUENCE = None


def conv_kernel_name(mode, d):
    bm, bn = ctypes.c_int(0), ctypes.c_int(0)
    lib().call('contrad_conv2d_tile', ctypes.byref(d), mode, ctypes.byref(bm), ctypes.byref(bn))
    path = lib().raw('contrad_conv2d_path')(ctypes.byref(d), mode)
    if path == 4:
        return 'wgrad_c32_kernel'
    if path == 5:
        return 'fwd_k1_kernel'
    if path == 6:
        return 'conv_c32_kernel<%d>' % mode
    if path == 7:
        return 'wino_wgrad_kernel' if mode == 2 else 'wino_kernel<%d>' % mode
    if path == 8:
        return 'wino22_wgrad_kernel' if mode == 2 else 'wino22_kernel<%d>' % mode
    if path == 9:
        return 'wino44_kernel<%d>' % mode
    if path == 11:
        return 'wino44n_kernel<%d>' % mode
    if path == 10:
        return 'wino23_kernel'
    if path in (2, 3):
        return 'igemm_lean_kernel<%d, %d, %d>' % (mode, bm.value, bn.value)
    return 'igemm_kernel<%d, %d, %d, %s>' % (mode, bm.value, bn.value, 'true' if path == 1 else 'false')


def _conv_call(mode, d, name, *args):
    if SEQUENCE is not None:
        SEQUENCE.append([conv_kernel_name(mode, d), [d.N, d.H, d.W, d.C, d.K, d.KH, d.KW, d.stride, d.pad],
                         int(lib().raw('contrad_conv2d_grid_blocks')(ctypes.byref(d), mode, 1)),
                         round(2.0 * d.N * d.Ho * d.Wo * d.K * d.C * d.KH * d.KW / 1e9, 4),
                         round(float(lib().raw('contrad_conv2d_executed_fraction')(ctypes.byref(d), mode)), 4)])
    if PROFILE is None:
        lib().call(name, *args)
        return
    kname = conv_kernel_name(mode, d)
    if PROFILE_ONLY is not None and kname != PROFILE_ONLY:
        lib().call(name, *args)
        return
    e0, e1 = torch.cuda.Event(enable_timing=True), torch.cuda.Event(enable_timing=True)
    st = torch.cuda.current_stream()
    e0.record(st)
    lib().call(name, *args)
    e1.record(st)
    flops = 2.0 * d.N * d.Ho * d.Wo * d.K * d.C * d.KH * d.KW
    shape = (d.N, d.H, d.W, d.C, d.K, d.KH, d.KW, d.stride, d.pad)
    blocks = lib().raw('contrad_conv2d_grid_blocks')(ctypes.byref(d), mode, 1)
    executed = float(lib().raw('contrad_conv2d_executed_fraction')(ctypes.byref(d), mode))
    PROFILE.append((kname, flops, e0, e1, shape, int(blocks), executed))


def make_desc(N, H, W, C, K, KH, KW, stride, pad, ldx, ldy, ldw):
    return ConvDesc(N, H, W, C, ldx, out_size(H, KH, stride, pad), out_size(W, KW, stride, pad), K, ldy,
                    KH, KW, stride, pad, ldw)


def pack_weight(w):
    K, C, KH, KW = w.shape
    ldw = round_up(K, 4)
    wp = w.new_zeros(KH * KW * C, ldw)
    wp[:, :K] = w.permute(2, 3, 1, 0).reshape(KH * KW * C, K)
    return wp


def unpack_weight(wp, K, C, KH, KW):
    return wp[:, :K].reshape(KH, KW, C, K).permute(3, 2, 0, 1).contiguous()


FILTER_PREP = os.environ.get('CONTRAD_DEV_FILTER_PREP', '1') != '0'
CONTRAST_PAIR = os.environ.get('CONTRAD_DEV_CONTRAST_PAIR', '1') != '0'
BN_FUSED = os.environ.get('CONTRAD_DEV_BN_FUSED', '1') != '0'


def filter_kind(d, mode):
    nb = ctypes.c_longlong(0)
    kind = lib().raw('contrad_conv2d_filter_kind')(ctypes.byref(d), mode, ctypes.byref(nb))
    if kind < 0:
        raise RuntimeError('contrad_hip: bad conv descriptor (%d)' % kind)
    return kind, nb.value


def fwd_desc(x_shape, wp, K, KH, KW, stride, pad):
    N, H, W, C = x_shape
    return make_desc(N, H, W, C, K, KH, KW, stride, pad, C, K, wp.stride(0))


def dgrad_desc(x_shape, wp, K, KH, KW, stride, pad):
    return fwd_desc(x_shape, wp, K, KH, KW, stride, pad)


class PreparedFilters(object):

    def __init__(self):
        self.jobs = {}
        self.buf = None

    def get(self, mode, wp):
        return self.jobs.get((mode, wp.data_ptr()))


def filter_prep(requests, device):
    pf = PreparedFilters()
    todo, tot = [], 0
    for mode, d, wp in requests:
        kind, nb = filter_kind(d, mode)
        if kind == 0 or (mode, wp.data_ptr()) in pf.jobs:
            continue
        _chk(wp, 'wp')
        j = FilterJob(wp.data_ptr(), 0, kind, mode, d.C, d.K, d.ldw)
        pf.jobs[(mode, wp.data_ptr())] = j
        todo.append((j, tot))
        tot += round_up(nb // 4, 4)
    if not todo:
        return pf
    pf.buf = torch.empty(tot, device=device, dtype=torch.float32)
    base = pf.buf.data_ptr()
    for j, off in todo:
        j.U = base + 4 * off
    for start in range(0, len(todo), FILTER_MAX_JOBS):
        b = FilterBatch()
        chunk = todo[start:start + FILTER_MAX_JOBS]
        b.n = len(chunk)
        for i, (j, _) in enumerate(chunk):
            b.jobs[i] = j
        lib().call('contrad_conv2d_filter_prep', ctypes.byref(b), _stream())
    return pf


def conv2d_fwd(x, wp, bias, K, KH, KW, stride, pad, slope=1.0, gain=1.0, out=None, addend=None, filters=None):
    _chk(x, 'x'); _chk(wp, 'wp'); _chk(bias, 'bias'); _chk(addend, 'addend')
    N, H, W, C = x.shape
    Ho, Wo = out_size(H, KH, stride, pad), out_size(W, KW, stride, pad)
    if out is None:
        out = torch.empty((N, Ho, Wo, K), device=x.device, dtype=torch.float32)
    _chk(out, 'out')
    d = make_desc(N, H, W, C, K, KH, KW, stride, pad, _ld(x), _ld(out), wp.stride(0))
    nbytes = lib().raw('contrad_conv2d_fwd_workspace_bytes')(ctypes.byref(d))
    ws = _workspace(nbytes, x.device) if nbytes > 0 else None
    if addend is not None and (tuple(addend.shape) != tuple(out.shape) or _ld(addend) != _ld(out)):
        raise RuntimeError('contrad_hip: addend must match y in shape and leading dimension')
    u = filters.get(0, wp) if filters is not None else None
    if u is not None:
        _conv_call(0, d, 'contrad_conv2d_fwd_add_u', ctypes.byref(d), _p(x), _p(wp), _p(bias), _p(addend), _p(out),
                   float(slope), float(gain), _p(ws), nbytes, ctypes.byref(u), _stream())
        return out
    _conv_call(0, d, 'contrad_conv2d_fwd_add', ctypes.byref(d), _p(x), _p(wp), _p(bias), _p(addend), _p(out),
               float(slope), float(gain), _p(ws), nbytes, _stream())
    return out


def conv2d_dgrad(gy, wp, x_shape, KH, KW, stride, pad, act_ref=None, slope=1.0, gain=1.0, out=None, filters=None):
    _chk(gy, 'gy'); _chk(wp, 'wp'); _chk(act_ref, 'act_ref')
    N, H, W, C = x_shape
    K = gy.shape[3]
    if out is None:
        out = torch.empty((N, H, W, C), device=gy.device, dtype=torch.float32)
    _chk(out, 'out')
    if act_ref is not None and (tuple(act_ref.shape) != tuple(out.shape) or _ld(act_ref) != _ld(out)):
        raise RuntimeError('contrad_hip: act_ref must match dx in shape and leading dimension')
    d = make_desc(N, H, W, C, K, KH, KW, stride, pad, _ld(out), _ld(gy), wp.stride(0))
    if (d.Ho, d.Wo) != (gy.shape[1], gy.shape[2]):
        raise RuntimeError('contrad_hip: gy spatial size does not match the conv geometry')
    nbytes = lib().raw('contrad_conv2d_dgrad_workspace_bytes')(ctypes.byref(d))
    ws = _workspace(nbytes, gy.device) if nbytes > 0 else None
    u = filters.get(1, wp) if filters is not None else None
    if u is not None:
        _conv_call(1, d, 'contrad_conv2d_dgrad_ws_u', ctypes.byref(d), _p(gy), _p(wp), _p(out), _p(act_ref),
                   float(slope), float(gain), _p(ws), nbytes, ctypes.byref(u), _stream())
        return out
    _conv_call(1, d, 'contrad_conv2d_dgrad_ws', ctypes.byref(d), _p(gy), _p(wp), _p(out), _p(act_ref),
               float(slope), float(gain), _p(ws), nbytes, _stream())
    return out


def conv2d_wino(mode, inp, wp, C, K, bias=None, ref=None, slope=1.0, gain=1.0, out=None, k4s2=False, f44=False, k3s2=False):
    _chk(inp, 'inp'); _chk(wp, 'wp'); _chk(bias, 'bias'); _chk(ref, 'ref')
    N, Hi, Wi, _ = inp.shape
    co = K if mode == 0 else C
    if k3s2:
        if mode != 0:
            raise RuntimeError('contrad_hip: the 3x3 stride-2 Winograd kernel is forward only')
        H, W = Hi, Wi
        oshape = (N, (H - 1) // 2, (W - 1) // 2, co)
        geo = (3, 3, 2, 0)
    elif k4s2:
        H, W = (Hi, Wi) if mode == 0 else (2 * Hi, 2 * Wi)
        oshape = (N, H // 2, W // 2, co) if mode == 0 else (N, H, W, co)
        geo = (4, 4, 2, 1)
    else:
        H, W = Hi, Wi
        oshape = (N, H, W, co)
        geo = (3, 3, 1, 1)
    if out is None:
        out = torch.empty(oshape, device=inp.device, dtype=torch.float32)
    _chk(out, 'out')
    if ref is not None and (tuple(ref.shape) != tuple(out.shape) or _ld(ref) != _ld(out)):
        raise RuntimeError('contrad_hip: ref must match the output in shape and leading dimension')
    d = make_desc(N, H, W, C, K, geo[0], geo[1], geo[2], geo[3], _ld(inp) if mode == 0 else _ld(out),
                  _ld(out) if mode == 0 else _ld(inp), wp.stride(0))
    if f44:
        if k4s2 or lib().raw('contrad_conv2d_wino44_ok')(ctypes.byref(d), mode) != 1:
            raise RuntimeError('contrad_hip: shape not supported by the F(4x4, 3x3) Winograd kernel')
        nbytes = lib().raw('contrad_conv2d_wino44_workspace_bytes')(ctypes.byref(d))
    else:
        if lib().raw('contrad_conv2d_wino_ok')(ctypes.byref(d), mode) != 1:
            raise RuntimeError('contrad_hip: shape not supported by the Winograd kernels')
        nbytes = lib().raw('contrad_conv2d_wino_workspace_bytes')(ctypes.byref(d), mode)
    if nbytes < 0:
        raise RuntimeError('contrad_hip: the Winograd workspace query rejected the shape (%d)' % nbytes)
    ws = _workspace(nbytes, inp.device)
    lib().call('contrad_conv2d_wino44' if f44 else 'contrad_conv2d_wino', ctypes.byref(d), mode, _p(inp), _p(wp), _p(bias), _p(ref), _p(out),
               float(slope), float(gain), _p(ws), ctypes.c_longlong(nbytes), _stream())
    return out


def conv2d_wino_wgrad(x, gy, ldw=None, out=None, dbias=None):
    _chk(x, 'x'); _chk(gy, 'gy')
    N, H, W, C = x.shape
    K = gy.shape[3]
    k, st = (3, 1) if gy.shape[1] == H else (4, 2)
    if out is None:
        out = torch.zeros((k * k * C, ldw or round_up(K, 4)), device=x.device, dtype=torch.float32)
    _chk(out, 'out')
    d = make_desc(N, H, W, C, K, k, k, st, 1, _ld(x), _ld(gy), out.stride(0))
    if lib().raw('contrad_conv2d_wino_ok')(ctypes.byref(d), 2) != 1:
        raise RuntimeError('contrad_hip: shape not supported by the Winograd weight-gradient kernel')
    nbytes = lib().raw('contrad_conv2d_wino_workspace_bytes')(ctypes.byref(d), 2)
    if nbytes < 0:
        raise RuntimeError('contrad_hip: the Winograd workspace query rejected the shape (%d)' % nbytes)
    ws = _workspace(nbytes, x.device)
    lib().call('contrad_conv2d_wino_wgrad', ctypes.byref(d), _p(x), _p(gy), _p(out), _p(dbias), _p(ws),
               ctypes.c_longlong(ws.numel() * 4), _stream())
    return out


_ws_cache = {}


class private_workspace(object):

    def __init__(self, owner_dict):
        self.mine = owner_dict

    def __enter__(self):
        global _ws_cache
        self.saved, _ws_cache = _ws_cache, self.mine
        return self

    def __exit__(self, *exc):
        global _ws_cache
        _ws_cache = self.saved
        return False


def _workspace(nbytes, device):
    key = (device.index, _stream_handle())
    buf = _ws_cache.get(key)
    if buf is None or buf.numel() * 4 < nbytes:
        buf = torch.empty((max(nbytes, 1) + 3) // 4, device=device, dtype=torch.float32)
        _ws_cache[key] = buf
    return buf


def conv2d_wgrad(x, gy, KH, KW, stride, pad, ldw=None, out=None, dbias=None):
    _chk(x, 'x'); _chk(gy, 'gy')
    N, H, W, C = x.shape
    K = gy.shape[3]
    if out is None:
        ldw = ldw or round_up(K, 4)
        out = torch.zeros((KH * KW * C, ldw), device=x.device, dtype=torch.float32)
    _chk(out, 'out')
    d = make_desc(N, H, W, C, K, KH, KW, stride, pad, _ld(x), _ld(gy), out.stride(0))
    nbytes = lib().raw('contrad_conv2d_wgrad_workspace_bytes')(ctypes.byref(d))
    if nbytes < 0:
        raise RuntimeError('contrad_hip: bad conv descriptor (%d)' % nbytes)
    ws = _workspace(nbytes, x.device)
    _conv_call(2, d, 'contrad_conv2d_wgrad', ctypes.byref(d), _p(x), _p(gy), _p(out), _p(dbias), _p(ws),
               ctypes.c_longlong(ws.numel() * 4), _stream())
    return out


def l2norm_fwd(u):
    _chk(u, 'u')
    R, D = u.shape
    z = torch.empty((R, D), device=u.device, dtype=torch.float32)
    inv = torch.empty((R,), device=u.device, dtype=torch.float32)
    lib().call('contrad_l2norm_fwd', _p(u), _ld(u), _p(z), _p(inv), R, D, 1e-12, _stream())
    return z, inv


def l2norm_bwd(dz, z, inv, out=None, accumulate=False):
    R, D = z.shape
    if out is None:
        out = torch.empty((R, D), device=z.device, dtype=torch.float32)
    lib().call('contrad_l2norm_bwd', _p(dz), _p(z), _p(inv), _p(out), _ld(out), R, D, int(accumulate), _stream())
    return out


def contrast_fwd(z, N, mode, temperature):
    _chk(z, 'z')
    if not z.is_contiguous():
        raise RuntimeError('contrad_hip: z must be contiguous')
    R, D = z.shape
    lse = torch.empty((R,), device=z.device, dtype=torch.float32)
    rowloss = torch.empty((R,), device=z.device, dtype=torch.float32)
    loss = torch.empty((1,), device=z.device, dtype=torch.float32)
    nbytes = lib().raw('contrad_contrast_workspace_bytes')(R, D)
    ws = _workspace(nbytes, z.device)
    lib().call('contrad_contrast_fwd', _p(z), R, D, N, mode, 1.0 / temperature, _p(lse), _p(rowloss), _p(loss),
               _p(ws), nbytes, _stream())
    return loss, lse


def contrast_bwd(z, lse, N, mode, temperature, grad_scale=None):
    R, D = z.shape
    dz = torch.empty((R, D), device=z.device, dtype=torch.float32)
    nbytes = lib().raw('contrad_contrast_workspace_bytes')(R, D)
    ws = _workspace(nbytes, z.device)
    lib().call('contrad_contrast_bwd', _p(z), _p(lse), R, D, N, mode, 1.0 / temperature, _p(grad_scale), _p(dz),
               _p(ws), nbytes, _stream())
    return dz


def l2norm_fwd_pair(u1, u2):
    probs = (L2normProblem * 2)()
    outs = []
    for q, u in zip(probs, (u1, u2)):
        _chk(u, 'u')
        R, D = u.shape
        z = torch.empty((R, D), device=u.device, dtype=torch.float32)
        inv = torch.empty((R,), device=u.device, dtype=torch.float32)
        q.u, q.ldu, q.z, q.inv_norm, q.R, q.D = u.data_ptr(), _ld(u), z.data_ptr(), inv.data_ptr(), R, D
        outs += [z, inv]
    lib().call('contrad_l2norm_fwd_batched', probs, 2, 1e-12, _stream())
    return tuple(outs)


def l2norm_bwd_pair(items):
    probs = (L2normProblem * 2)()
    for q, (dz, z, inv, out, zero_rows) in zip(probs, items):
        R, D = z.shape
        q.dz, q.z, q.inv_norm, q.du = dz.data_ptr(), z.data_ptr(), inv.data_ptr(), out.data_ptr()
        q.ldu, q.R, q.D, q.accumulate, q.zero_rows = _ld(out), R, D, 0, int(zero_rows)
    lib().call('contrad_l2norm_bwd_batched', probs, 2, _stream())


def _contrast_pair(items, temperature):
    probs = (ContrastProblem * 2)()
    sizes = []
    for z, N, mode in items:
        _chk(z, 'z')
        if not z.is_contiguous():
            raise RuntimeError('contrad_hip: z must be contiguous')
        sizes.append(round_up(lib().raw('contrad_contrast_workspace_bytes')(z.shape[0], z.shape[1]), 16))
    ws = _workspace(sum(sizes), items[0][0].device)
    off = 0
    for q, (z, N, mode), nb in zip(probs, items, sizes):
        q.z, q.R, q.D, q.N, q.mode, q.inv_temp = z.data_ptr(), z.shape[0], z.shape[1], N, mode, 1.0 / temperature
        q.workspace, q.workspace_bytes = ws.data_ptr() + off, nb
        off += nb
    return probs, ws


def contrast_fwd_pair(z1, N1, mode1, z2, N2, mode2, temperature):
    probs, ws = _contrast_pair(((z1, N1, mode1), (z2, N2, mode2)), temperature)
    outs = []
    for q, z in zip(probs, (z1, z2)):
        R = z.shape[0]
        lse = torch.empty((R,), device=z.device, dtype=torch.float32)
        rowloss = torch.empty((R,), device=z.device, dtype=torch.float32)
        loss = torch.empty((1,), device=z.device, dtype=torch.float32)
        q.lse, q.rowloss, q.loss = lse.data_ptr(), rowloss.data_ptr(), loss.data_ptr()
        outs += [loss, lse, rowloss]
    lib().call('contrad_contrast_fwd_batched', probs, 2, _stream())
    return outs[0], outs[1], outs[3], outs[4]


def contrast_bwd_pair(z1, lse1, N1, mode1, gs1, z2, lse2, N2, mode2, gs2, temperature):
    probs, ws = _contrast_pair(((z1, N1, mode1), (z2, N2, mode2)), temperature)
    outs = []
    for q, z, lse, gs in zip(probs, (z1, z2), (lse1, lse2), (gs1, gs2)):
        dz = torch.empty(tuple(z.shape), device=z.device, dtype=torch.float32)
        q.lse, q.grad_scale, q.dz = lse.data_ptr(), (gs.data_ptr() if gs is not None else None), dz.data_ptr()
        outs.append(dz)
    lib().call('contrad_contrast_bwd_batched', probs, 2, _stream())
    return outs[0], outs[1]


from ._lib import SnBatch, SnLayer, AdamBatch, SN_MAX_LAYERS, ADAM_MAX_TENSORS, AUG_NPARAM


class SnSpec(object):
    __slots__ = ('w', 'u', 'v', 'K', 'C', 'T', 'fixed_scale')

    def __init__(self, w, u=None, v=None, fixed_scale=0.0, view_kct=None):
        self.w, self.u, self.v = w, u, v
        if view_kct is not None:
            self.K, self.C, self.T = view_kct
        elif w.dim() == 4:
            self.K, self.C, self.T = w.shape[0], w.shape[1], w.shape[2] * w.shape[3]
        else:
            self.K, self.C, self.T = w.shape[0], w.shape[1], 1
        assert self.K * self.C * self.T == w.numel()
        self.fixed_scale = float(fixed_scale)


def sn_scratch_floats(specs):
    offs, tot = [], 0
    for s in specs:
        offs.append(tot)
        tot += int(lib().raw('contrad_sn_scratch_floats')(s.K, s.C, s.T))
        tot = round_up(tot, 4)
    return offs, tot


def _sn_batches(specs, wps, ldws, offs, u_snaps=None, v_snaps=None, gwps=None, gws=None):
    for start in range(0, len(specs), SN_MAX_LAYERS):
        b = SnBatch()
        chunk = specs[start:start + SN_MAX_LAYERS]
        b.n = len(chunk)
        for j, s in enumerate(chunk):
            i = start + j
            L = b.layers[j]
            L.w = s.w.data_ptr()
            L.u = s.u.data_ptr() if s.u is not None else None
            L.v = s.v.data_ptr() if s.v is not None else None
            L.u_snap = u_snaps[i].data_ptr() if (u_snaps is not None and u_snaps[i] is not None) else None
            L.v_snap = v_snaps[i].data_ptr() if (v_snaps is not None and v_snaps[i] is not None) else None
            L.wp = wps[i].data_ptr()
# ... 521 lines not shown
```

### contrad_amd/training/gan/contrad.py

```python
import torch
import torch.distributed as dist

from ... import ops
from ...third_party.gather_layer import GatherLayer, all_gather_rows
from ..criterion import _Contrast, MODE_NT_XENT, MODE_SUPCON_FAKE


def supcon_fake(out1, out2, others, temperature, distributed=False):
    if distributed:
        out1 = torch.cat(GatherLayer.apply(out1), dim=0)
        out2 = torch.cat(GatherLayer.apply(out2), dim=0)
        others = torch.cat(GatherLayer.apply(others), dim=0)
    N = out1.size(0)
    return _Contrast.apply(torch.cat([out1, out2, others], dim=0), N, MODE_SUPCON_FAKE, temperature)


def _regroup(gathered, blocks, n):
    W, _, D = gathered.shape
    return gathered.view(W, blocks, n, D).transpose(0, 1).reshape(blocks * W * n, D)


class _ContraDContrastive(torch.autograd.Function):

    @staticmethod
    def forward(ctx, proj, proj2, N, temperature, distributed):
        D = proj.shape[1]
        from ...engine import dist_on
        world, rank = 1, 0
        gathered = distributed and dist_on()
        if not gathered and ops.CONTRAST_PAIR:
            z1, inv1, z2, inv2 = ops.l2norm_fwd_pair(proj[:2 * N], proj2)
            l1, lse1, l2, lse2 = ops.contrast_fwd_pair(z1, N, MODE_NT_XENT, z2, N, MODE_SUPCON_FAKE, temperature)
            ctx.save_for_backward(z1, inv1, z2, inv2, z1, z2, lse1, lse2)
            ctx.cfg = (N, N, temperature, world, rank, tuple(proj.shape), D)
            return l1.reshape(()), l2.reshape(())
        z1, inv1 = ops.l2norm_fwd(proj[:2 * N])
        z2, inv2 = ops.l2norm_fwd(proj2)
        if gathered:
            world, rank = dist.get_world_size(), dist.get_rank()
            packed = torch.cat([z1, z2], dim=0)
            g = all_gather_rows(packed)
            z1g = _regroup(g[:, :2 * N], 2, N)
            z2g = _regroup(g[:, 2 * N:], 3, N)
        else:
            z1g, z2g = z1, z2
        Ng = N * world
        l1, lse1 = ops.contrast_fwd(z1g, Ng, MODE_NT_XENT, temperature)
        l2, lse2 = ops.contrast_fwd(z2g, Ng, MODE_SUPCON_FAKE, temperature)
        ctx.save_for_backward(z1, inv1, z2, inv2, z1g, z2g, lse1, lse2)
        ctx.cfg = (N, Ng, temperature, world, rank, tuple(proj.shape), D)
        return l1.reshape(()), l2.reshape(())

    @staticmethod
    def backward(ctx, g1, g2):
        z1, inv1, z2, inv2, z1g, z2g, lse1, lse2 = ctx.saved_tensors
        N, Ng, temperature, world, rank, pshape, D = ctx.cfg
        if world == 1 and ops.CONTRAST_PAIR:
            gs1, gs2 = g1.reshape(1).contiguous().float(), g2.reshape(1).contiguous().float()
            dz1, dz2 = ops.contrast_bwd_pair(z1g, lse1, Ng, MODE_NT_XENT, gs1, z2g, lse2, Ng, MODE_SUPCON_FAKE, gs2,
                                             temperature)
            dproj = torch.empty(pshape, device=z1.device, dtype=torch.float32)
            dproj2 = torch.empty(pshape, device=z1.device, dtype=torch.float32)
            ops.l2norm_bwd_pair(((dz1, z1, inv1, dproj[:2 * N], pshape[0] - 2 * N), (dz2, z2, inv2, dproj2, 0)))
            return dproj, dproj2, None, None, None
        dz1 = ops.contrast_bwd(z1g, lse1, Ng, MODE_NT_XENT, temperature, g1.reshape(1).contiguous().float())
        dz2 = ops.contrast_bwd(z2g, lse2, Ng, MODE_SUPCON_FAKE, temperature, g2.reshape(1).contiguous().float())
        if world > 1:
            dz1 = dz1.view(2, world, N, D)[:, rank].reshape(2 * N, D).contiguous()
            dz2 = dz2.view(3, world, N, D)[:, rank].reshape(3 * N, D).contiguous()
        dproj = torch.zeros(pshape, device=z1.device, dtype=torch.float32)
        ops.l2norm_bwd(dz1, z1, inv1, out=dproj[:2 * N])
        dproj2 = ops.l2norm_bwd(dz2, z2, inv2)
        return dproj, dproj2, None, None, None


class _GanDLoss(torch.autograd.Function):

    @staticmethod
    def forward(ctx, d_all, N, kind):
        out, grad = ops.gan_d_loss(d_all.contiguous(), N, kind)
        ctx.save_for_backward(grad)
        loss, d_real, d_gen = out.unbind(0)
        ctx.mark_non_differentiable(d_real, d_gen)
        return loss, d_real, d_gen

    @staticmethod
    def backward(ctx, g, _g1, _g2):
        grad, = ctx.saved_tensors
        return grad * g, None, None


class _GanGLoss(torch.autograd.Function):
    @staticmethod
    def forward(ctx, d_gen, kind):
        out, grad = ops.gan_g_loss(d_gen.contiguous(), kind)
        ctx.save_for_backward(grad)
        return out[0]

    @staticmethod
    def backward(ctx, g):
        grad, = ctx.saved_tensors
        return grad * g, None


_D_LOSSES = ('nonsat', 'wgan', 'hinge', 'lsgan')


def loss_D_fn(P, D, options, images, gen_images):
    assert images.size(0) == gen_images.size(0)
    if options['loss'] not in _D_LOSSES:
        raise NotImplementedError()
    gen_images = gen_images.detach()
    N = images.size(0)

    cat_images = torch.cat([images, images, gen_images], dim=0)
    d_all, aux = D(P.augment_fn(cat_images), sg_linear=True, projection=True, projection2=True)
    simclr_loss, sup_loss = _ContraDContrastive.apply(aux['projection'], aux['projection2'], N, P.temp,
                                                      bool(P.distributed))
    d_loss, d_real, d_gen = _GanDLoss.apply(d_all, N, options['loss'])
    return simclr_loss + P.lbd_a * sup_loss, {
        "penalty": d_loss,
        "d_real": d_real,
        "d_gen": d_gen,
    }


def loss_G_fn(P, D, options, images, gen_images):
    d_gen = D(P.augment_fn(gen_images))
    return _GanGLoss.apply(d_gen, options['loss'])
```

### include/contrad_hip.h

```cpp
#ifndef CONTRAD_HIP_H
#define CONTRAD_HIP_H

#ifdef __cplusplus
extern "C" {
#endif

typedef void* contrad_stream_t;

int contrad_abi_version(void);

typedef struct {
  int N, H, W, C;
  int ldx;
  int Ho, Wo, K;
  int ldy;
  int KH, KW;
  int stride, pad;
  int ldw;
} contrad_conv_desc;

int contrad_conv2d_fwd(const contrad_conv_desc* d, const float* x, const float* wp, const float* bias,
                       float* y, float slope, float gain, float* workspace, long long workspace_bytes,
                       contrad_stream_t stream);
int contrad_conv2d_fwd_add(const contrad_conv_desc* d, const float* x, const float* wp, const float* bias,
                           const float* addend, float* y, float slope, float gain, float* workspace,
                           long long workspace_bytes, contrad_stream_t stream);
long long contrad_conv2d_fwd_workspace_bytes(const contrad_conv_desc* d);

int contrad_conv2d_dgrad(const contrad_conv_desc* d, const float* gy, const float* wp, float* dx,
                         const float* act_ref, float slope, float gain, contrad_stream_t stream);
long long contrad_conv2d_dgrad_workspace_bytes(const contrad_conv_desc* d);
int contrad_conv2d_dgrad_ws(const contrad_conv_desc* d, const float* gy, const float* wp, float* dx,
                            const float* act_ref, float slope, float gain, float* workspace,
                            long long workspace_bytes, contrad_stream_t stream);

int contrad_conv2d_wino_ok(const contrad_conv_desc* d, int mode);
long long contrad_conv2d_wino_workspace_bytes(const contrad_conv_desc* d, int mode);
int contrad_conv2d_wino_wgrad(const contrad_conv_desc* d, const float* x, const float* gy, float* dwp, float* dbias,
                              float* workspace, long long workspace_bytes, contrad_stream_t stream);
int contrad_conv2d_wino(const contrad_conv_desc* d, int mode, const float* in, const float* wp, const float* bias,
                        const float* ref, float* out, float slope, float gain, float* workspace,
                        long long workspace_bytes, contrad_stream_t stream);

int contrad_conv2d_wino44_ok(const contrad_conv_desc* d, int mode);
long long contrad_conv2d_wino44_workspace_bytes(const contrad_conv_desc* d);
int contrad_conv2d_wino44(const contrad_conv_desc* d, int mode, const float* in, const float* wp, const float* bias,
                          const float* ref, float* out, float slope, float gain, float* workspace,
                          long long workspace_bytes, contrad_stream_t stream);

#define CONTRAD_FILTER_MAX_JOBS 16
typedef struct {
  const float* wp;
  float* U;
  int kind;
  int mode;
  int C, K, ldw;
} contrad_filter_job;
typedef struct {
  int n;
  contrad_filter_job jobs[CONTRAD_FILTER_MAX_JOBS];
  int block_start[CONTRAD_FILTER_MAX_JOBS + 1];
} contrad_filter_batch;
int contrad_conv2d_filter_kind(const contrad_conv_desc* d, int mode, long long* bytes);
int contrad_conv2d_filter_prep(const contrad_filter_batch* b, contrad_stream_t stream);
int contrad_conv2d_fwd_add_u(const contrad_conv_desc* d, const float* x, const float* wp, const float* bias,
                             const float* addend, float* y, float slope, float gain, float* workspace,
                             long long workspace_bytes, const contrad_filter_job* u, contrad_stream_t stream);
int contrad_conv2d_dgrad_ws_u(const contrad_conv_desc* d, const float* gy, const float* wp, float* dx,
                              const float* act_ref, float slope, float gain, float* workspace,
                              long long workspace_bytes, const contrad_filter_job* u, contrad_stream_t stream);

long long contrad_conv2d_wgrad_workspace_bytes(const contrad_conv_desc* d);
int contrad_conv2d_tile(const contrad_conv_desc* d, int mode, int* bm, int* bn);
int contrad_conv2d_path(const contrad_conv_desc* d, int mode);
double contrad_conv2d_executed_fraction(const contrad_conv_desc* d, int mode);
long long contrad_conv2d_grid_blocks(const contrad_conv_desc* d, int mode, int with_workspace);
int contrad_conv2d_tile_order(const contrad_conv_desc* d, int mode, unsigned char* out, int capacity);
int contrad_conv2d_wgrad(const contrad_conv_desc* d, const float* x, const float* gy, float* dwp,
                         float* dbias, float* workspace, long long workspace_bytes, contrad_stream_t stream);

long long contrad_contrast_workspace_bytes(int R, int D);
int contrad_contrast_fwd(const float* z, int R, int D, int N, int mode, float inv_temp, float* lse,
                         float* rowloss, float* loss, float* workspace, long long workspace_bytes,
                         contrad_stream_t stream);
int contrad_contrast_bwd(const float* z, const float* lse, int R, int D, int N, int mode, float inv_temp,
                         const float* grad_scale, float* dz, float* workspace, long long workspace_bytes,
                         contrad_stream_t stream);
int contrad_l2norm_fwd(const float* u, int ldu, float* z, float* inv_norm, int R, int D, float eps,
                       contrad_stream_t stream);
int contrad_l2norm_bwd(const float* dz, const float* z, const float* inv_norm, float* du, int ldu, int R,
                       int D, int accumulate, contrad_stream_t stream);

#define CONTRAD_CONTRAST_MAX_PROBLEMS 2
typedef struct {
  const float* z;
  int R, D, N, mode;
  float inv_temp;
  float* lse;
  float* rowloss;
  float* loss;
  const float* grad_scale;
  float* dz;
  float* workspace;
  long long workspace_bytes;
} contrad_contrast_problem;
int contrad_contrast_fwd_batched(const contrad_contrast_problem* p, int n, contrad_stream_t stream);
int contrad_contrast_bwd_batched(const contrad_contrast_problem* p, int n, contrad_stream_t stream);
typedef struct {
  const float* u;
  float* z;
  float* inv_norm;
  const float* dz;
  float* du;
  int ldu, R, D;
  int accumulate;
  int zero_rows;
} contrad_l2norm_problem;
int contrad_l2norm_fwd_batched(const contrad_l2norm_problem* p, int n, float eps, contrad_stream_t stream);
int contrad_l2norm_bwd_batched(const contrad_l2norm_problem* p, int n, contrad_stream_t stream);

#define CONTRAD_SN_MAX_LAYERS 24
#define CONTRAD_SN_MAX_PARTIALS 256
typedef struct {
  const float* w;
  float* u;
  float* v;
  float* u_snap;
  float* v_snap;
  float* wp;
  const float* gwp;
  float* gw;
  int K, C, T, ldw;
  float fixed_scale;
} contrad_sn_layer;
typedef struct {
  int n;
  contrad_sn_layer layers[CONTRAD_SN_MAX_LAYERS];
  long long scratch_off[CONTRAD_SN_MAX_LAYERS];
} contrad_sn_batch;

long long contrad_sn_scratch_floats(int K, int C, int T);
int contrad_sn_weight_prep(const contrad_sn_batch* b, int training, float eps, float* scratch,
                           float* sigma_out, contrad_stream_t stream);
int contrad_sn_weight_grad(const contrad_sn_batch* b, float* scratch, const float* sigma,
                           contrad_stream_t stream);

int contrad_rgb_conv_fwd(const float* img, const float* wp, const float* bias, float* y, int N, int Cin,
                         int H, int W, int K, int k, int ldy, int ldw, float in_scale, float in_shift,
                         float slope, float gain, contrad_stream_t stream);
long long contrad_rgb_conv_wgrad_workspace_bytes(int N, int Cin, int H, int W, int K, int k);
int contrad_rgb_conv_wgrad(const float* img, const float* gy, float* dwp, float* dbias, int N, int Cin,
                           int H, int W, int K, int k, int ldy, int ldw, float in_scale, float in_shift,
                           float* workspace, long long workspace_bytes, contrad_stream_t stream);
int contrad_rgb_conv_dgrad(const float* gy, const float* wp, const float* bias, const float* mod,
                           const float* residual, float* out, int N, int C, int H, int W, int K, int k,
                           int ldy, int ldw, int act, float out_scale, float out_shift,
                           contrad_stream_t stream);

long long contrad_colstats_workspace_bytes(long long M, int K, int with_sq);
int contrad_colstats(const float* x, long long M, int K, int ld, int with_sq, float* out, int accumulate,
                     float* workspace, long long workspace_bytes, contrad_stream_t stream);
int contrad_bn_relu_apply(const float* x, float* y, long long M, int K, int ldx, int ldy, const float* stats,
                          float count, const float* gamma, const float* beta, float eps, int perm_hw,
                          contrad_stream_t stream);
int contrad_bn_relu_bwd_stats(const float* dy, const float* x, long long M, int K, int ld, const float* stats,
                              float count, const float* gamma, const float* beta, float eps, float* out2k,
                              float* workspace, long long workspace_bytes, contrad_stream_t stream);
int contrad_bn_relu_bwd_apply(const float* dy, const float* x, float* dx, long long M, int K, int ld,
                              const float* stats, float count, const float* gamma, const float* beta, float eps,
                              const float* bstats, contrad_stream_t stream);
int contrad_bn_running_update(const float* stats, float count, int K, const float* conv_bias, float momentum,
                              float* running_mean, float* running_var, long long* num_batches_tracked,
                              contrad_stream_t stream);
int contrad_bn_batch_stats(const float* x, long long M, int K, int ld, float* stats, const float* conv_bias,
                           float momentum, float* running_mean, float* running_var, long long* num_batches_tracked,
                           float* workspace, long long workspace_bytes, contrad_stream_t stream);
int contrad_gan_d_loss(const float* logits, int ld, int N, int kind, float* out3, float* grad,
                       contrad_stream_t stream);
int contrad_gan_g_loss(const float* logits, int ld, int N, int kind, float* out1, float* grad,
                       contrad_stream_t stream);

#define CONTRAD_ADAM_MAX_TENSORS 64
#define CONTRAD_ADAM_CHUNK 16384
typedef struct {
  float* p;
  const float* g;
  float* m;
  float* v;
  long long numel;
} contrad_adam_tensor;
typedef struct {
  int n;
  contrad_adam_tensor t[CONTRAD_ADAM_MAX_TENSORS];
  int block_start[CONTRAD_ADAM_MAX_TENSORS + 1];
} contrad_adam_batch;
int contrad_adam_step(const contrad_adam_batch* b, int step, float lr, float beta1, float beta2, float eps,
                      float grad_scale, contrad_stream_t stream);
int contrad_adam_step_dev(const contrad_adam_batch* b, const float* hyper_dev, float beta1, float beta2, float eps,
                          contrad_stream_t stream);
int contrad_axpby(float* y, const float* x, long long n, float a, float b, contrad_stream_t stream);
int contrad_pull_host(const float* host_pinned, float* dst, long long n, contrad_stream_t stream);

#define CONTRAD_AUG_NPARAM 16
long long contrad_simclr_workspace_bytes(int B, int H, int W);
int contrad_simclr_augment(const float* x, float* y, const float* params, int B, int H, int W,
                           int contrast_first, int has_contrast, float* workspace,
                           long long workspace_bytes, contrad_stream_t stream);
long long contrad_simclr_augment_bwd_workspace_bytes(int B, int H, int W);
int contrad_simclr_augment_bwd(const float* x, const float* params, const float* grad_out, float* grad_in,
                               int B, int H, int W, int contrast_first, int has_contrast, float* workspace,
                               long long workspace_bytes, contrad_stream_t stream);
int contrad_gaussian_blur_masked(const float* x, float* tmp, float* y, const float* params,
                                 const float* kernel1d, int B, int H, int W, int radius,
                                 contrad_stream_t stream);
int contrad_cutout_masked(float* y, const float* params, int B, int H, int W, int length, contrad_stream_t stream);
int contrad_gaussian_blur_masked_bwd(const float* grad_out, float* tmp, float* grad_in, const float* params,
                                     const float* kernel1d, int B, int H, int W, int radius,
                                     contrad_stream_t stream);

int contrad_upfirdn2d(const float* input, const float* kernel, float* out, int major, int in_h, int in_w,
                      int minor, int kh, int kw, int up_x, int up_y, int down_x, int down_y, int pad_x0,
                      int pad_x1, int pad_y0, int pad_y1, contrad_stream_t stream);
int contrad_upfirdn2d_fused(const float* input, const float* kernel, float* out, int major, int in_h, int in_w,
                            int minor, int kh, int kw, int up_x, int up_y, int down_x, int down_y, int pad_x0,
                            int pad_x1, int pad_y0, int pad_y1, const float* addend, const float* act_ref, float slope,
                            float gain, float* out2, contrad_stream_t stream);
int contrad_fused_bias_act(const float* x, const float* bias, const float* ref, float* y, long long n,
                           int step_b, int size_b, int act, int grad, float alpha, float scale,
                           contrad_stream_t stream);
int contrad_lincomb(const float* x, const float* z, float* y, long long n, float a, float b,
                    contrad_stream_t stream);

// ... 60 lines not shown
```

Baseline: 47690 images/sec.

## Skip dead head-row rectangles in 1x1 head GEMMs across fwd, dgrad and wgrad

Adds masked variants of the 1x1 convolution forward, data-gradient and weight-gradient paths that take up to four dead row/column rectangles and skip the tiles or K-slices that fall inside them. The discriminator passes head row ranges so the logits head only computes rows for one real copy and the fakes, and the projection head only the real rows. This is meant to remove wasted GEMM work on outputs the loss never uses. The cost is extra planning logic, a masked reduce kernel that zeroes dead outputs, and new kernel instantiations.

```diff
diff --git a/contrad_amd/csrc/igemm.hip b/contrad_amd/csrc/igemm.hip
--- a/contrad_amd/csrc/igemm.hip
+++ b/contrad_amd/csrc/igemm.hip
@@ -45,7 +45,20 @@
   int pixmajor;
   int px_full;
   int st_nt;
+  int ndead;
+  int dead_r0[4], dead_r1[4], dead_c0[4], dead_c1[4];
 };
+
+__host__ __device__ inline void dead_span(const IgemmArgs& p, int i, bool cover_rows, int a_lo, int a_hi, int unit, int ext,
+                                          int* lo, int* hi) {
+  *lo = 0; *hi = 0;
+  if (i >= p.ndead) return;
+  const int x0 = cover_rows ? p.dead_r0[i] : p.dead_c0[i], x1 = cover_rows ? p.dead_r1[i] : p.dead_c1[i];
+  const int y0 = cover_rows ? p.dead_c0[i] : p.dead_r0[i], y1 = cover_rows ? p.dead_c1[i] : p.dead_r1[i];
+  if (!(x0 <= a_lo && a_hi <= x1)) return;
+  const int l = (y0 + unit - 1) / unit, h = (y1 >= ext) ? (ext + unit - 1) / unit : y1 / unit;
+  if (h > l) { *lo = l; *hi = h; }
+}
 
 constexpr long long NT_STORE_BYTES = 256ll << 20;
 inline int st_nt_for(long long rows, int ld) {
@@ -2380,3 +2393,299 @@
   CONTRAD_CHECK_LAUNCH();
   return 0;
 }
+
+namespace {
+
+__global__ void fwd_reduce_masked_kernel(const IgemmArgs p, const float* __restrict__ ws, int splits,
+                                         float* __restrict__ y, int only_dead) {
+  const long long M = p.M;
+  const int Ncol = p.Ncol, ldy = p.d.ldy;
+  const long long total = M * Ncol;
+  for (long long e = (long long)blockIdx.x * blockDim.x + threadIdx.x; e < total;
+       e += (long long)gridDim.x * blockDim.x) {
+    const long long m = e / Ncol;
+    const int c = (int)(e - m * Ncol);
+    bool dead = false;
+#pragma unroll
+    for (int i = 0; i < 4; ++i)
+      dead = dead || (i < p.ndead && m >= p.dead_r0[i] && m < p.dead_r1[i] && c >= p.dead_c0[i] && c < p.dead_c1[i]);
+    if (dead) { y[m * ldy + c] = 0.f; continue; }
+    if (only_dead) continue;
+    float v = 0.f;
+    for (int k = 0; k < splits; ++k) v += ws[(long long)k * total + e];
+    if (p.bias) v += p.bias[c];
+    v = (v > 0.f) ? v : v * p.slope;
+    v *= p.gain;
+    y[m * ldy + c] = v;
+  }
+}
+
+template <int MODE, int BM, int BN>
+int launch_lean_dead_inst(const IgemmArgs& a, dim3 grid, hipStream_t stream) {
+  static bool attr_set_dev[64] = {};
+  constexpr size_t smem = lean_smem_bytes<MODE, BM, BN>();
+  int dev_id = 0;
+  (void)hipGetDevice(&dev_id);
+  bool& attr_set = attr_set_dev[dev_id & 63];
+  if (!attr_set) {
+    hipError_t e = hipFuncSetAttribute(reinterpret_cast<const void*>(&igemm_lean_dead_kernel<MODE, BM, BN>),
+                                       hipFuncAttributeMaxDynamicSharedMemorySize, (int)smem);
+    if (e != hipSuccess) return (int)e;
+    attr_set = true;
+  }
+  IgemmArgs b = a;
+  b.ny = (int)grid.y;
+  hipLaunchKernelGGL((igemm_lean_dead_kernel<MODE, BM, BN>), dim3(grid.x * grid.y), dim3(NTHREADS), smem, stream, b);
+  CONTRAD_CHECK_LAUNCH();
+  return 0;
+}
+
+IgemmArgs snap_to_tiles(const IgemmArgs& a, int bm, int bn, int M, int Ncol) {
+  IgemmArgs s = a;
+  for (int i = 0; i < a.ndead; ++i) {
+    s.dead_r0[i] = cdiv(a.dead_r0[i], bm) * bm;
+    s.dead_r1[i] = a.dead_r1[i] >= M ? M : a.dead_r1[i] / bm * bm;
+    s.dead_c0[i] = cdiv(a.dead_c0[i], bn) * bn;
+    s.dead_c1[i] = a.dead_c1[i] >= Ncol ? Ncol : a.dead_c1[i] / bn * bn;
+  }
+  return s;
+}
+
+bool dead_tile_ok(int bm, int bn) { return (bm == 128 || bm == 64) && (bn == 128 || bn == 64); }
+
+template <int MODE>
+int launch_lean_dead(const IgemmArgs& a, int bm, int bn, dim3 grid, hipStream_t s) {
+  if (bm == 128 && bn == 128) return launch_lean_dead_inst<MODE, 128, 128>(a, grid, s);
+  if (bm == 128 && bn == 64) return launch_lean_dead_inst<MODE, 128, 64>(a, grid, s);
+  if (bm == 64 && bn == 128) return launch_lean_dead_inst<MODE, 64, 128>(a, grid, s);
+  if (bm == 64 && bn == 64) return launch_lean_dead_inst<MODE, 64, 64>(a, grid, s);
+  return -22;
+}
+
+struct DeadPlan {
+  bool masked;
+  int bm, bn, tiles_m, tiles_n, splits, tps;
+  long long live_units, all_units;
+  long long blocks;
+  unsigned char order[256];
+};
+
+int dead_plan(const contrad_conv_desc* d, int mode, const int* dead, int n_dead, bool may_split, IgemmArgs* a, DeadPlan* pl) {
+  int rc = check_desc(d);
+  if (rc) return rc;
+  CONTRAD_ARG(mode >= 0 && mode <= 2 && n_dead >= 1 && n_dead <= 4 && dead != nullptr);
+  CONTRAD_ARG(d->H == 1 && d->W == 1 && d->KH == 1 && d->KW == 1 && d->stride == 1 && d->pad == 0);
+  for (int i = 0; i < n_dead; ++i) {
+    const int* r = dead + 4 * i;
+    CONTRAD_ARG(0 <= r[0] && r[0] < r[1] && r[1] <= d->N && 0 <= r[2] && r[2] < r[3] && r[3] <= d->K);
+    for (int j = 0; j < i; ++j) {
+      const int* q = dead + 4 * j;
+      CONTRAD_ARG(!(r[0] < q[1] && q[0] < r[1] && r[2] < q[3] && q[2] < r[3]));
+    }
+    a->dead_r0[i] = r[0]; a->dead_r1[i] = r[1]; a->dead_c0[i] = r[2]; a->dead_c1[i] = r[3];
+  }
+  a->ndead = n_dead;
+  a->d = *d;
+  pl->live_units = pl->all_units = 0;
+  pl->masked = contrad_conv2d_path(d, mode) == 2;
+  if (!pl->masked) return 0;
+  if (mode == MODE_FWD) {
+    const FwdPlan p = fwd_plan(d);
+    if (!dead_tile_ok(p.bm, p.bn)) { pl->masked = false; return 0; }
+    pl->bm = p.bm; pl->bn = p.bn; pl->splits = p.splits; pl->tps = p.tps;
+    pl->tiles_m = cdiv(d->N, p.bm); pl->tiles_n = cdiv(d->K, p.bn);
+    for (int tm = 0; tm < pl->tiles_m; ++tm) {
+      int live = pl->tiles_n;
+      for (int i = 0; i < 4; ++i) {
+        int lo, hi;
+        dead_span(*a, i, true, tm * p.bm, std::min(tm * p.bm + p.bm, d->N), p.bn, d->K, &lo, &hi);
+        live -= hi - lo;
+      }
+      pl->live_units += live;
+    }
+    pl->all_units = (long long)pl->tiles_m * pl->tiles_n;
+    pl->blocks = pl->live_units * p.splits;
+  } else if (mode == MODE_DGRAD) {
+    const FwdPlan p = dgrad_plan(d, may_split);
+    pl->bm = p.bm; pl->bn = p.bn; pl->splits = p.splits; pl->tps = p.tps;
+    pl->tiles_m = cdiv(d->N, p.bm); pl->tiles_n = cdiv(d->C, p.bn);
+    if (!dead_tile_ok(p.bm, p.bn) || pl->tiles_m > 256) { pl->masked = false; return 0; }
+    const int kt = d->K / BK;
+    int work[256];
+    for (int tm = 0; tm < pl->tiles_m; ++tm) {
+      int live = kt;
+      for (int i = 0; i < 4; ++i) {
+        int lo, hi;
+        dead_span(*a, i, true, tm * p.bm, std::min(tm * p.bm + p.bm, d->N), BK, d->K, &lo, &hi);
+        live -= hi - lo;
+      }
+      work[tm] = live;
+      pl->live_units += (long long)live * pl->tiles_n;
+    }
+    pl->all_units = (long long)kt * pl->tiles_m * pl->tiles_n;
+    pl->blocks = (long long)pl->tiles_m * pl->tiles_n * p.splits;
+    pixel_order(work, pl->tiles_m, pl->order);
+  } else {
+    int pps;
+    wgrad_plan(d, &pl->bm, &pl->bn, &pl->tiles_m, &pl->tiles_n, &pl->splits, &pps);
+    if (!dead_tile_ok(pl->bm, pl->bn)) { pl->masked = false; return 0; }
+    pl->tps = pps;
+    const int pt = d->N / BK;
+    for (int tn = 0; tn < pl->tiles_n; ++tn) {
+      int live = pt;
+      for (int i = 0; i < 4; ++i) {
+        int lo, hi;
+        dead_span(*a, i, false, tn * pl->bn, std::min(tn * pl->bn + pl->bn, d->K), BK, d->N, &lo, &hi);
+        live -= hi - lo;
+      }
+      pl->live_units += (long long)live * pl->tiles_m;
+    }
+    pl->all_units = (long long)pt * pl->tiles_m * pl->tiles_n;
+    pl->blocks = (long long)pl->tiles_m * pl->tiles_n * pl->splits;
+  }
+  return 0;
+}
+
+}
+
+extern "C" int contrad_conv2d_path_masked(const contrad_conv_desc* d, int mode, const int* dead, int n_dead) {
+  if (n_dead == 0) return contrad_conv2d_path(d, mode);
+  IgemmArgs a{};
+  DeadPlan pl;
+  if (dead_plan(d, mode, dead, n_dead, true, &a, &pl)) return -22;
+  return pl.masked ? 12 : contrad_conv2d_path(d, mode);
+}
+
+extern "C" double contrad_conv2d_executed_fraction_masked(const contrad_conv_desc* d, int mode, const int* dead,
+                                                          int n_dead) {
+  if (n_dead == 0) return contrad_conv2d_executed_fraction(d, mode);
+  IgemmArgs a{};
+  DeadPlan pl;
+  if (dead_plan(d, mode, dead, n_dead, true, &a, &pl)) return -22.0;
+  if (!pl.masked) return contrad_conv2d_executed_fraction(d, mode);
+  return (double)pl.live_units / (double)pl.all_units;
+}
+
+extern "C" long long contrad_conv2d_grid_blocks_masked(const contrad_conv_desc* d, int mode, int with_workspace,
+                                                       const int* dead, int n_dead) {
+  if (n_dead == 0) return contrad_conv2d_grid_blocks(d, mode, with_workspace);
+  IgemmArgs a{};
+  DeadPlan pl;
+  if (dead_plan(d, mode, dead, n_dead, with_workspace != 0, &a, &pl)) return -22;
+  if (!pl.masked) return contrad_conv2d_grid_blocks(d, mode, with_workspace);
+  if (mode == MODE_FWD && !with_workspace) return pl.live_units;
+  return pl.blocks;
+}
+
+extern "C" int contrad_conv2d_fwd_masked(const contrad_conv_desc* d, const float* x, const float* wp, const float* bias,
+                                         float* y, float slope, float gain, float* workspace, long long workspace_bytes,
+                                         const int* dead, int n_dead, contrad_stream_t stream) {
+  if (n_dead == 0) return contrad_conv2d_fwd(d, x, wp, bias, y, slope, gain, workspace, workspace_bytes, stream);
+  IgemmArgs a{};
+  DeadPlan pl;
+  int rc = dead_plan(d, MODE_FWD, dead, n_dead, true, &a, &pl);
+  if (rc) return rc;
+  a.M = d->N; a.Ncol = d->K; a.Kg = d->C;
+  if (!pl.masked) {
+    rc = contrad_conv2d_fwd(d, x, wp, bias, y, slope, gain, workspace, workspace_bytes, stream);
+    if (rc) return rc;
+    int bm = 0, bn = 0;
+    contrad_conv2d_tile(d, MODE_FWD, &bm, &bn);
+    const long long total = (long long)d->N * d->K;
+    hipLaunchKernelGGL(fwd_reduce_masked_kernel, dim3((unsigned)std::min<long long>((total + 255) / 256, 2048)), dim3(256),
+                       0, (hipStream_t)stream, snap_to_tiles(a, bm, bn, d->N, d->K), workspace, 1, y, 1);
+    CONTRAD_CHECK_LAUNCH();
+    return 0;
+  }
+  CONTRAD_ARG(x && wp && y && aligned16(x, wp, y));
+  a.A = x; a.B = wp; a.C = y; a.bias = bias; a.slope = slope; a.gain = gain;
+  a.st_nt = st_nt_for(d->N, d->ldy);
+  a.tiles_m = pl.tiles_m; a.tiles_n = pl.tiles_n; a.ptiles_per_split = pl.tps;
+  if (pl.splits > 1) {
+    CONTRAD_ARG(workspace && workspace_bytes >= contrad_conv2d_fwd_workspace_bytes(d));
+    a.C = workspace;
+  }
+  if (pl.live_units > 0) {
+    rc = launch_lean_dead<MODE_FWD>(a, pl.bm, pl.bn, dim3((unsigned)pl.live_units, pl.splits), (hipStream_t)stream);
+    if (rc) return rc;
+  }
+  const long long total = (long long)d->N * d->K;
+  int blocks = (int)((total + 255) / 256);
+  if (blocks > 2048) blocks = 2048;
+  hipLaunchKernelGGL(fwd_reduce_masked_kernel, dim3(blocks), dim3(256), 0, (hipStream_t)stream,
+                     snap_to_tiles(a, pl.bm, pl.bn, d->N, d->K), workspace, pl.splits, y, pl.splits > 1 ? 0 : 1);
+  CONTRAD_CHECK_LAUNCH();
+  return 0;
+}
+
+extern "C" int contrad_conv2d_dgrad_masked(const contrad_conv_desc* d, const float* gy, const float* wp, float* dx,
+                                           const float* act_ref, float slope, float gain, float* workspace,
+                                           long long workspace_bytes, const int* dead, int n_dead,
+                                           contrad_stream_t stream) {
+  if (n_dead == 0) return contrad_conv2d_dgrad_ws(d, gy, wp, dx, act_ref, slope, gain, workspace, workspace_bytes, stream);
+  IgemmArgs a{};
+  DeadPlan pl;
+  int rc = dead_plan(d, MODE_DGRAD, dead, n_dead, workspace != nullptr, &a, &pl);
+  if (rc) return rc;
+  if (!pl.masked)
+    return contrad_conv2d_dgrad_ws(d, gy, wp, dx, act_ref, slope, gain, workspace, workspace_bytes, stream);
+  CONTRAD_ARG(gy && wp && dx && aligned16(gy, wp, dx) && aligned16(act_ref, nullptr, nullptr));
+  a.A = gy; a.B = wp; a.C = dx; a.act_ref = act_ref; a.slope = slope; a.gain = gain;
+  a.st_nt = st_nt_for(d->N, d->ldx);
+  a.px_pixels = 1;
+  a.tiles_m = pl.tiles_m; a.tiles_n = pl.tiles_n;
+  memcpy(a.px_order, pl.order, sizeof(a.px_order));
+  const dim3 grid(pl.tiles_m * pl.tiles_n, pl.splits);
+  if (pl.splits <= 1) return launch_lean_dead<MODE_DGRAD>(a, pl.bm, pl.bn, grid, (hipStream_t)stream);
+  CONTRAD_ARG(workspace_bytes >= contrad_conv2d_dgrad_workspace_bytes(d));
+  a.dsplits = pl.splits;
+  a.ptiles_per_split = pl.tps;
+  a.slab_elems = (long long)d->N * d->ldx;
+  a.C = workspace; a.act_ref = nullptr;
+  rc = launch_lean_dead<MODE_DGRAD>(a, pl.bm, pl.bn, grid, (hipStream_t)stream);
+  if (rc) return rc;
+  const long long rows = d->N;
+  long long blocks = (rows * (d->C / 4) + 255) / 256;
+  if (blocks > 4096) blocks = 4096;
+  hipLaunchKernelGGL(dgrad_reduce_kernel, dim3((unsigned)blocks), dim3(256), 0, (hipStream_t)stream, workspace,
+                     pl.splits, a.slab_elems, rows, d->C, d->ldx, act_ref, slope, gain, dx);
+  CONTRAD_CHECK_LAUNCH();
+  return 0;
+}
+
+extern "C" int contrad_conv2d_wgrad_masked(const contrad_conv_desc* d, const float* x, const float* gy, float* dwp,
+                                           float* dbias, float* workspace, long long workspace_bytes, const int* dead,
+                                           int n_dead, contrad_stream_t stream) {
+  if (n_dead == 0) return contrad_conv2d_wgrad(d, x, gy, dwp, dbias, workspace, workspace_bytes, stream);
+  IgemmArgs a{};
+  DeadPlan pl;
+  int rc = dead_plan(d, MODE_WGRAD, dead, n_dead, true, &a, &pl);
+  if (rc) return rc;
+  if (!pl.masked) return contrad_conv2d_wgrad(d, x, gy, dwp, dbias, workspace, workspace_bytes, stream);
+  CONTRAD_ARG(x && gy && dwp && workspace && aligned16(x, gy, workspace));
+  CONTRAD_ARG(workspace_bytes >= contrad_conv2d_wgrad_workspace_bytes(d));
+  const int splits = pl.splits;
+  a.tiles_m = pl.tiles_m; a.tiles_n = pl.tiles_n;
+  a.A = x; a.B = gy; a.C = workspace;
+  a.M = d->C; a.Ncol = d->K; a.Kg = a.M;
+  a.bias_ws = dbias ? workspace + (size_t)splits * a.M * a.Ncol : nullptr;
+  a.P = d->N; a.ptiles_per_split = pl.tps;
+  a.pixmajor = wgrad_pixmajor_ok(d, pl.bm, pl.tps) ? 1 : 0;
+  const bool direct = splits == 1 && d->ldw == d->K;
+  if (direct) {
+    a.C = dwp;
+    if (dbias) a.bias_ws = dbias;
+  }
+  rc = launch_lean_dead<MODE_WGRAD>(a, pl.bm, pl.bn, dim3(a.tiles_m * a.tiles_n, splits), (hipStream_t)stream);
+  if (rc || direct) return rc;
+  const long long total = (long long)a.M * a.Ncol;
+  int R = 1;
+  while (R < 64 && R * 2 <= splits && (total / 4) * R < 65536) R <<= 1;
+  long long blocks = ((total / 4) * R + 255) / 256;
+  if (blocks > 2048) blocks = 2048;
+  if (blocks < 1) blocks = 1;
+  hipLaunchKernelGGL(wgrad_reduce_kernel, dim3((int)blocks), dim3(256), 0, (hipStream_t)stream, workspace, dwp,
+                     a.M, a.Ncol, d->ldw, splits, a.bias_ws, dbias, R);
+  CONTRAD_CHECK_LAUNCH();
+  return 0;
+}
diff --git a/contrad_amd/csrc/igemm_lean.h b/contrad_amd/csrc/igemm_lean.h
--- a/contrad_amd/csrc/igemm_lean.h
+++ b/contrad_amd/csrc/igemm_lean.h
@@ -34,11 +34,12 @@
   else { q = x / d; r = x - q * d; }
 }
 
-template <int MODE, int BM, int BN, bool BAL>
+template <int MODE, int BM, int BN, bool BAL, bool DEAD = false>
 __device__ __forceinline__ void lean_tile(const IgemmArgs& p, float* smem, const int tile_m, const int tile_n, const int by,
                                           const int wc_h0, const int wc_w0, const int wc_hc, const int wc_wc) {
   static_assert(BK == 16, "the lean loop is written for a 16-deep K-tile");
   static_assert(!BAL || MODE == MODE_DGRAD, "balanced order: strided data gradient only");
+  static_assert(!DEAD || !BAL, "dead rectangles: 1x1 layers only");
   const int pl_pixmajor = BAL ? 0 : p.pixmajor, pl_nwin = BAL ? 0 : p.nwin, pl_dsplits = BAL ? 0 : p.dsplits;
   constexpr bool A_Q = (MODE != MODE_WGRAD);
   constexpr bool B_Q = (MODE == MODE_DGRAD);
@@ -81,6 +82,31 @@
   int u_n = 0, u_h = 0, u_w = 0;
   int ph = 0, pw = 0, Hc = 0, Wc = 0, kh0 = 0, kw0 = 0, nth = 0, ntw = 1, bh = 0, bw = 0;
   int gw = 1, gh = 1, gn = 1, n_begin = 0;
+  int dk_lo[4] = {0, 0, 0, 0}, dk_hi[4] = {0, 0, 0, 0}, u_t = 0;
+  auto dead_kt = [&](int t) -> bool {
+    bool r = false;
+#pragma unroll
+    for (int i = 0; i < 4; ++i) r = r || (t >= dk_lo[i] && t < dk_hi[i]);
+    return r;
+  };
+  auto dead_trim = [&](int t_begin) -> int {
+    int live = T, first = t_begin;
+#pragma unroll
+    for (int i = 0; i < 4; ++i) live -= max(0, min(dk_hi[i], t_begin + T) - max(dk_lo[i], t_begin));
+#pragma unroll
+    for (int r = 0; r < 4; ++r)
+#pragma unroll
+      for (int i = 0; i < 4; ++i)
+        if (first >= dk_lo[i] && first < dk_hi[i]) first = dk_hi[i];
+    if (live <= 0) {
+#pragma unroll
+      for (int i = 0; i < 4; ++i) { dk_lo[i] = 0; dk_hi[i] = 0; }
+      live = 0; first = t_begin;
+    }
+    T = live;
+    u_t = first;
+    return first;
+  };
 
   if constexpr (MODE == MODE_FWD) {
     const int t_total = p.Kg / BK, t_begin = by * p.ptiles_per_split;
@@ -190,6 +216,11 @@
       u_a = u_tap / ntw;
       u_b = u_tap - u_a * ntw;
     }
+    if constexpr (DEAD) {
+#pragma unroll
+      for (int i = 0; i < 4; ++i) dead_span(p, i, true, m0, min(m0 + BM, M), BK, d.K, &dk_lo[i], &dk_hi[i]);
+      u_c0 = dead_trim(pl_dsplits > 1 ? by * p.ptiles_per_split : 0) * BK;
+    }
     if (ntw == 0) ntw = 1;
     if (pl_nwin > 0) {
       Hc = wc_hc; Wc = wc_wc;
@@ -275,9 +306,14 @@
     }
   } else {
     const int tiles_total = p.P / BK;
-    const int t_begin = by * p.ptiles_per_split;
+    int t_begin = by * p.ptiles_per_split;
     T = min(p.ptiles_per_split, tiles_total - t_begin);
     if (T < 0) T = 0;
+    if constexpr (DEAD) {
+#pragma unroll
+      for (int i = 0; i < 4; ++i) dead_span(p, i, false, n0, min(n0 + BN, Ncol), BK, p.P, &dk_lo[i], &dk_hi[i]);
+      t_begin = dead_trim(t_begin);
+    }
     gw = min(d.Wo, 16);
     gh = min(d.Ho, 16 / gw);
     if (pl_pixmajor) { gw = 1; gh = 1; }
@@ -401,7 +437,8 @@
           u_b = 0; ++u_a; pos_offA += wk_ah; pos_offB += wk_bh;
           if (u_a == nth) { u_a = 0; u_tap = 0; pos_offA += wk_an; pos_offB += wk_bn; }
         }
-      } while (!((tapmask >> u_tap) & 1u));
+        if constexpr (DEAD) ++u_t;
+      } while (!((tapmask >> u_tap) & 1u) || (DEAD && dead_kt(u_t)));
     } else {
       do {
         u_w += gw; pos_offA += wk_aw; pos_offB += wk_b;
@@ -410,7 +447,8 @@
           if (u_h == d.Ho) { u_h = 0; u_n += gn; pos_offA += wk_an; pos_offB += wk_bn; }
         }
         pos_edge = wgrad_pos_edge();
-      } while (wskip & pos_edge);
+        if constexpr (DEAD) ++u_t;
+      } while ((wskip & pos_edge) || (DEAD && dead_kt(u_t)));
     }
   };
   auto load_a_piece = [&](int set, int i) {
@@ -831,6 +869,51 @@
 }
 
 template <int MODE, int BM, int BN>
+__global__ __launch_bounds__(NTHREADS, IGEMM_MIN_WAVES) void igemm_lean_dead_kernel(const IgemmArgs p) {
+  extern __shared__ __attribute__((aligned(16))) float smem[];
+  int by = 0, tile_n = 0, tile_m = 0;
+  if constexpr (MODE == MODE_FWD) {
+    int rem = xcd_remap(blockIdx.x, gridDim.x);
+    bool found = false;
+    for (int tm = 0; tm < p.tiles_m && !found; ++tm) {
+      int lo[4], hi[4], live = p.tiles_n;
+#pragma unroll
+      for (int i = 0; i < 4; ++i) {
+        dead_span(p, i, true, tm * BM, min(tm * BM + BM, p.M), BN, p.Ncol, &lo[i], &hi[i]);
+        live -= hi[i] - lo[i];
+      }
+      if (rem >= live * p.ny) { rem -= live * p.ny; continue; }
+      by = rem / live;
+      int j = rem - by * live;
+      for (int tn = 0; tn < p.tiles_n; ++tn) {
+        bool dead = false;
+#pragma unroll
+        for (int i = 0; i < 4; ++i) dead = dead || (tn >= lo[i] && tn < hi[i]);
+        if (dead) continue;
+        if (j == 0) { tile_n = tn; break; }
+        --j;
+      }
+      tile_m = tm;
+      found = true;
+    }
+    if (!found) return;
+  } else if constexpr (MODE == MODE_DGRAD) {
+    const int lin = blockIdx.x;
+    tile_n = lin % p.tiles_n;
+    const int r = lin / p.tiles_n;
+    by = r % p.ny;
+    tile_m = p.px_order[r / p.ny];
+  } else {
+    const int lin = xcd_remap(blockIdx.x, gridDim.x);
+    const int tiles = p.tiles_m * p.tiles_n;
+    by = lin / tiles;
+    const int b = lin - by * tiles;
+    tile_n = b % p.tiles_n; tile_m = b / p.tiles_n;
+  }
+  lean_tile<MODE, BM, BN, false, MODE != MODE_FWD>(p, smem, tile_m, tile_n, by, 0, 0, 0, 0);
+}
+
+template <int MODE, int BM, int BN>
 constexpr size_t lean_smem_bytes() {
   const int a = (MODE != MODE_WGRAD) ? 4 * (BM * 4 + LEAN_QPAD) : 16 * BM;
   const int b = (MODE == MODE_DGRAD) ? 4 * (BN * 4 + LEAN_QPAD) : 16 * (BN < 64 ? 64 : BN);
diff --git a/contrad_amd/engine.py b/contrad_amd/engine.py
--- a/contrad_amd/engine.py
+++ b/contrad_amd/engine.py
@@ -265,13 +265,13 @@
 
     def _body(self):
         from . import ops
-        from .training.gan.contrad import _ContraDContrastive, _GanDLoss
+        from .training.gan.contrad import _ContraDContrastive, _GanDLoss, d_head_rows
         P, G, D, N = self.P, self.G, self.D, self.N
         with torch.no_grad():
             gen = G(self.z)
             cat = torch.cat([self.images, self.images, gen], dim=0)
             aug = ops.simclr_augment(cat, self.params, -1, self.aug.r_c is not None)
-        d_all, aux = D(aug, sg_linear=True, projection=True, projection2=True)
+        d_all, aux = D(aug, sg_linear=True, projection=True, projection2=True, _head_rows=d_head_rows(N))
         simclr, sup = _ContraDContrastive.apply(aux['projection'], aux['projection2'], N, P.temp,
                                                 bool(P.distributed) and self.dist)
         gan, d_real, d_gen = _GanDLoss.apply(d_all, N, self.options['loss'])
diff --git a/contrad_amd/models/gan/base.py b/contrad_amd/models/gan/base.py
--- a/contrad_amd/models/gan/base.py
+++ b/contrad_amd/models/gan/base.py
@@ -131,7 +131,7 @@
         raise NotImplementedError
 
     def forward(self, inputs, y=None, penultimate=False, projection=False, projection2=False,
-                finetuning=False, sg_linear=False):
+                finetuning=False, sg_linear=False, _head_rows=None):
         if y is not None:
             raise NotImplementedError('class-conditional heads (n_classes > 1) are not used by get_architecture')
         lin = self._modules.get('linear')
@@ -140,6 +140,9 @@
         if getattr(self, '_lazy_projections', False):
             output, project, project2, features = self._run(inputs, sg_linear, finetuning, want_features,
                                                             want_proj=(projection or projection2))
+        elif _head_rows is not None and getattr(self, '_takes_head_rows', False) and not replaced:
+            output, project, project2, features = self._run(inputs, sg_linear, finetuning, want_features,
+                                                            head_rows=_head_rows)
         else:
             output, project, project2, features = self._run(inputs, sg_linear, finetuning, want_features)
         if replaced:
diff --git a/contrad_amd/models/gan/sndcgan.py b/contrad_amd/models/gan/sndcgan.py
--- a/contrad_amd/models/gan/sndcgan.py
+++ b/contrad_amd/models/gan/sndcgan.py
@@ -63,7 +63,7 @@
 
 class _DFunction(torch.autograd.Function):
     @staticmethod
-    def forward(ctx, D, images, sg_linear, want_features, trunk_grad, *params):
+    def forward(ctx, D, images, sg_linear, want_features, trunk_grad, dead_rows, *params):
         dev = images.device
         plan = _DPlan(D, dev)
         specs = plan.specs
@@ -109,7 +109,8 @@
             x = ops.conv2d_fwd(x, wps[i], biases[i], co, k, k, s, p, _SLOPE, 1.0, filters=filters)
             acts.append(x)
         bias_cat = torch.cat([biases[7], biases[8], biases[9]])
-        hidden = ops.conv2d_fwd(x.view(B, 1, 1, plan.feat), merged, bias_cat, 3 * dh, 1, 1, 1, 0, _SLOPE, 1.0)
+        dead = tuple((r0, r1, j * dh, (j + 1) * dh) for j, rows in enumerate(dead_rows) for (r0, r1) in rows)
+        hidden = ops.conv2d_fwd(x.view(B, 1, 1, plan.feat), merged, bias_cat, 3 * dh, 1, 1, 1, 0, _SLOPE, 1.0, dead=dead)
         logits = ops.conv2d_fwd(hidden[..., 0:dh], wps[10], biases[10], 1, 1, 1, 1, 0).view(B, 1)
         proj = ops.conv2d_fwd(hidden[..., dh:2 * dh], wps[11], biases[11], dp, 1, 1, 1, 0).view(B, dp)
         proj2 = ops.conv2d_fwd(hidden[..., 2 * dh:3 * dh], wps[12], biases[12], dp, 1, 1, 1, 0).view(B, dp)
@@ -120,7 +121,7 @@
         ctx.images, ctx.acts, ctx.hidden = images, acts, hidden
         ctx.wps, ctx.ldws, ctx.merged, ctx.wbuf, ctx.filters = wps, ldws, merged, wbuf, filters
         ctx.sigma, ctx.u_snaps, ctx.v_snaps, ctx.snapbuf = sigma, u_snaps, v_snaps, snapbuf
-        ctx.sg_linear, ctx.trunk_grad = sg_linear, trunk_grad
+        ctx.sg_linear, ctx.trunk_grad, ctx.dead = sg_linear, trunk_grad, dead
         ctx.param_shapes = [tuple(p.shape) for p in params]
         if want_features:
             feats = x.permute(0, 3, 1, 2).reshape(B, -1)
@@ -138,7 +139,7 @@
         B = images.shape[0]
         dh, dp = plan.dh, plan.dp
         n = len(specs)
-        need_params = any(ctx.needs_input_grad[5:])
+        need_params = any(ctx.needs_input_grad[6:])
         need_images = ctx.needs_input_grad[1]
         a6 = acts[6]
         comm = getattr(D, '_grad_comm', None)
@@ -185,7 +186,8 @@
             o7 = gbias[7].storage_offset()
             adjacent = all(gbias[7 + j].storage_offset() == o7 + j * dh for j in range(3))
             gb_hidden = bbuf[o7:o7 + 3 * dh] if adjacent else torch.empty(3 * dh, device=dev, dtype=torch.float32)
-            ops.conv2d_wgrad(a6.view(B, 1, 1, plan.feat), g_hidden, 1, 1, 1, 0, out=gmerged, dbias=gb_hidden)
+            ops.conv2d_wgrad(a6.view(B, 1, 1, plan.feat), g_hidden, 1, 1, 1, 0, out=gmerged, dbias=gb_hidden,
+                             dead=ctx.dead)
             exchange(gmerged)
             if not adjacent:
                 for j in range(3):
@@ -194,9 +196,10 @@
         if ctx.trunk_grad:
             lo = dh if ctx.sg_linear else 0
             fused = g_feats is None or g_feats.numel() == 0
+            dead_lo = tuple((r0, r1, c0 - lo, c1 - lo) for (r0, r1, c0, c1) in ctx.dead if c0 >= lo)
             g = ops.conv2d_dgrad(g_hidden[..., lo:], ctx.merged[:, lo:], (B, 1, 1, plan.feat), 1, 1, 1, 0,
                                  act_ref=a6.view(B, 1, 1, plan.feat) if fused else None, slope=_SLOPE,
-                                 gain=1.0).view(a6.shape)
+                                 gain=1.0, dead=dead_lo).view(a6.shape)
             if not fused:
                 g = g + g_feats.reshape(B, 512, plan.hb, plan.wb).permute(0, 2, 3, 1)
                 g = (g * torch.where(a6 > 0, 1.0, _SLOPE)).contiguous()
@@ -231,7 +234,7 @@
             for i in range(n):
                 grads[2 * i] = gws[i].view(ctx.param_shapes[2 * i])
                 grads[2 * i + 1] = gbias[i]
-        return (None, d_images, None, None, None) + tuple(grads)
+        return (None, d_images, None, None, None, None) + tuple(grads)
 
 
 class D_SNDCGAN(BaseDiscriminator):
@@ -269,14 +272,36 @@
             out += [m.weight_orig, m.bias]
         return out
 
-    def _run(self, inputs, sg_linear, finetuning, want_features):
+    _takes_head_rows = True
+
+    @staticmethod
+    def _dead_rows(head_rows, B):
+        out = []
+        for key in ('logits', 'projection', 'projection2'):
+            live = sorted((int(a), int(b)) for a, b in head_rows[key]) if head_rows and key in head_rows else [(0, B)]
+            gaps, at = [], 0
+            for a, b in live:
+                if not (0 <= a <= b <= B) or a < at:
+                    raise ValueError('head rows of %s: ranges must be ascending, disjoint and inside the batch' % key)
+                if a > at:
+                    gaps.append((at, a))
+                at = b
+            if at < B:
+                gaps.append((at, B))
+            out.append(tuple(gaps))
+        if sum(len(g) for g in out) > 4:
+            return ((), (), ())
+        return tuple(out)
+
+    def _run(self, inputs, sg_linear, finetuning, want_features, head_rows=None):
         if not inputs.is_cuda:
             raise RuntimeError('contrad_amd.D_SNDCGAN runs on the MI355X HIP path only (no CPU fallback)')
         if finetuning:
             inputs = inputs.detach()
         images = inputs.contiguous().float()
+        dead_rows = self._dead_rows(head_rows, images.shape[0]) if head_rows is not None else ((), (), ())
         logits, proj, proj2, feats = _DFunction.apply(self, images, bool(sg_linear), bool(want_features),
-                                                      not finetuning, *self._ordered_params())
+                                                      not finetuning, dead_rows, *self._ordered_params())
         return logits, proj, proj2, (feats if want_features else None)
 
     def penultimate(self, inputs):
diff --git a/contrad_amd/ops.py b/contrad_amd/ops.py
--- a/contrad_amd/ops.py
+++ b/contrad_amd/ops.py
@@ -57,10 +57,21 @@
 SEQUENCE = None
 
 
-def conv_kernel_name(mode, d):
+def _dead_table(dead):
+    dead = tuple(tuple(int(v) for v in r) for r in (dead or ()))
+    if not dead:
+        return None, 0
+    flat = [v for r in dead for v in r]
+    return (ctypes.c_int * len(flat))(*flat), len(dead)
+
+
+def conv_kernel_name(mode, d, dead=None):
     bm, bn = ctypes.c_int(0), ctypes.c_int(0)
     lib().call('contrad_conv2d_tile', ctypes.byref(d), mode, ctypes.byref(bm), ctypes.byref(bn))
-    path = lib().raw('contrad_conv2d_path')(ctypes.byref(d), mode)
+    tab, nd = _dead_table(dead)
+    path = lib().raw('contrad_conv2d_path_masked')(ctypes.byref(d), mode, tab, nd)
+    if path == 12:
+        return 'igemm_lean_dead_kernel<%d, %d, %d>' % (mode, bm.value, bn.value)
     if path == 4:
         return 'wgrad_c32_kernel'
     if path == 5:
@@ -82,16 +93,17 @@
     return 'igemm_kernel<%d, %d, %d, %s>' % (mode, bm.value, bn.value, 'true' if path == 1 else 'false')
 
 
-def _conv_call(mode, d, name, *args):
+def _conv_call(mode, d, name, *args, dead=None):
+    tab, nd = _dead_table(dead)
     if SEQUENCE is not None:
-        SEQUENCE.append([conv_kernel_name(mode, d), [d.N, d.H, d.W, d.C, d.K, d.KH, d.KW, d.stride, d.pad],
-                         int(lib().raw('contrad_conv2d_grid_blocks')(ctypes.byref(d), mode, 1)),
+        SEQUENCE.append([conv_kernel_name(mode, d, dead), [d.N, d.H, d.W, d.C, d.K, d.KH, d.KW, d.stride, d.pad],
+                         int(lib().raw('contrad_conv2d_grid_blocks_masked')(ctypes.byref(d), mode, 1, tab, nd)),
                          round(2.0 * d.N * d.Ho * d.Wo * d.K * d.C * d.KH * d.KW / 1e9, 4),
-                         round(float(lib().raw('contrad_conv2d_executed_fraction')(ctypes.byref(d), mode)), 4)])
+                         round(float(lib().raw('contrad_conv2d_executed_fraction_masked')(ctypes.byref(d), mode, tab, nd)), 4)])
     if PROFILE is None:
         lib().call(name, *args)
         return
-    kname = conv_kernel_name(mode, d)
+    kname = conv_kernel_name(mode, d, dead)
     if PROFILE_ONLY is not None and kname != PROFILE_ONLY:
         lib().call(name, *args)
         return
@@ -102,8 +114,8 @@
     e1.record(st)
     flops = 2.0 * d.N * d.Ho * d.Wo * d.K * d.C * d.KH * d.KW
     shape = (d.N, d.H, d.W, d.C, d.K, d.KH, d.KW, d.stride, d.pad)
-    blocks = lib().raw('contrad_conv2d_grid_blocks')(ctypes.byref(d), mode, 1)
-    executed = float(lib().raw('contrad_conv2d_executed_fraction')(ctypes.byref(d), mode))
+    blocks = lib().raw('contrad_conv2d_grid_blocks_masked')(ctypes.byref(d), mode, 1, tab, nd)
+    executed = float(lib().raw('contrad_conv2d_executed_fraction_masked')(ctypes.byref(d), mode, tab, nd))
     PROFILE.append((kname, flops, e0, e1, shape, int(blocks), executed))
 
 
@@ -184,7 +196,7 @@
     return pf
 
 
-def conv2d_fwd(x, wp, bias, K, KH, KW, stride, pad, slope=1.0, gain=1.0, out=None, addend=None, filters=None):
+def conv2d_fwd(x, wp, bias, K, KH, KW, stride, pad, slope=1.0, gain=1.0, out=None, addend=None, filters=None, dead=None):
     _chk(x, 'x'); _chk(wp, 'wp'); _chk(bias, 'bias'); _chk(addend, 'addend')
     N, H, W, C = x.shape
     Ho, Wo = out_size(H, KH, stride, pad), out_size(W, KW, stride, pad)
@@ -196,6 +208,13 @@
     ws = _workspace(nbytes, x.device) if nbytes > 0 else None
     if addend is not None and (tuple(addend.shape) != tuple(out.shape) or _ld(addend) != _ld(out)):
         raise RuntimeError('contrad_hip: addend must match y in shape and leading dimension')
+    if dead:
+        if addend is not None:
+            raise RuntimeError('contrad_hip: the masked forward takes no addend')
+        tab, nd = _dead_table(dead)
+        _conv_call(0, d, 'contrad_conv2d_fwd_masked', ctypes.byref(d), _p(x), _p(wp), _p(bias), _p(out), float(slope),
+                   float(gain), _p(ws), nbytes, tab, nd, _stream(), dead=dead)
+        return out
     u = filters.get(0, wp) if filters is not None else None
     if u is not None:
         _conv_call(0, d, 'contrad_conv2d_fwd_add_u', ctypes.byref(d), _p(x), _p(wp), _p(bias), _p(addend), _p(out),
@@ -206,7 +225,8 @@
     return out
 
 
-def conv2d_dgrad(gy, wp, x_shape, KH, KW, stride, pad, act_ref=None, slope=1.0, gain=1.0, out=None, filters=None):
+def conv2d_dgrad(gy, wp, x_shape, KH, KW, stride, pad, act_ref=None, slope=1.0, gain=1.0, out=None, filters=None,
+                 dead=None):
     _chk(gy, 'gy'); _chk(wp, 'wp'); _chk(act_ref, 'act_ref')
     N, H, W, C = x_shape
     K = gy.shape[3]
@@ -220,6 +240,11 @@
         raise RuntimeError('contrad_hip: gy spatial size does not match the conv geometry')
     nbytes = lib().raw('contrad_conv2d_dgrad_workspace_bytes')(ctypes.byref(d))
     ws = _workspace(nbytes, gy.device) if nbytes > 0 else None
+    if dead:
+        tab, nd = _dead_table(dead)
+        _conv_call(1, d, 'contrad_conv2d_dgrad_masked', ctypes.byref(d), _p(gy), _p(wp), _p(out), _p(act_ref),
+                   float(slope), float(gain), _p(ws), nbytes, tab, nd, _stream(), dead=dead)
+        return out
     u = filters.get(1, wp) if filters is not None else None
     if u is not None:
         _conv_call(1, d, 'contrad_conv2d_dgrad_ws_u', ctypes.byref(d), _p(gy), _p(wp), _p(out), _p(act_ref),
@@ -319,7 +344,7 @@
     return buf
 
 
-def conv2d_wgrad(x, gy, KH, KW, stride, pad, ldw=None, out=None, dbias=None):
+def conv2d_wgrad(x, gy, KH, KW, stride, pad, ldw=None, out=None, dbias=None, dead=None):
     _chk(x, 'x'); _chk(gy, 'gy')
     N, H, W, C = x.shape
     K = gy.shape[3]
@@ -332,6 +357,11 @@
     if nbytes < 0:
         raise RuntimeError('contrad_hip: bad conv descriptor (%d)' % nbytes)
     ws = _workspace(nbytes, x.device)
+    if dead:
+        tab, nd = _dead_table(dead)
+        _conv_call(2, d, 'contrad_conv2d_wgrad_masked', ctypes.byref(d), _p(x), _p(gy), _p(out), _p(dbias), _p(ws),
+                   ctypes.c_longlong(ws.numel() * 4), tab, nd, _stream(), dead=dead)
+        return out
     _conv_call(2, d, 'contrad_conv2d_wgrad', ctypes.byref(d), _p(x), _p(gy), _p(out), _p(dbias), _p(ws),
                ctypes.c_longlong(ws.numel() * 4), _stream())
     return out
diff --git a/contrad_amd/training/gan/contrad.py b/contrad_amd/training/gan/contrad.py
--- a/contrad_amd/training/gan/contrad.py
+++ b/contrad_amd/training/gan/contrad.py
@@ -103,6 +103,10 @@
         return grad * g, None
 
 
+def d_head_rows(N):
+    return {'logits': ((0, N), (2 * N, 3 * N)), 'projection': ((0, 2 * N),)}
+
+
 _D_LOSSES = ('nonsat', 'wgan', 'hinge', 'lsgan')
 
 
@@ -114,7 +118,8 @@
     N = images.size(0)
 
     cat_images = torch.cat([images, images, gen_images], dim=0)
-    d_all, aux = D(P.augment_fn(cat_images), sg_linear=True, projection=True, projection2=True)
+    d_all, aux = D(P.augment_fn(cat_images), sg_linear=True, projection=True, projection2=True,
+                   _head_rows=d_head_rows(N))
     simclr_loss, sup_loss = _ContraDContrastive.apply(aux['projection'], aux['projection2'], N, P.temp,
                                                       bool(P.distributed))
     d_loss, d_real, d_gen = _GanDLoss.apply(d_all, N, options['loss'])
diff --git a/include/contrad_hip.h b/include/contrad_hip.h
--- a/include/contrad_hip.h
+++ b/include/contrad_hip.h
@@ -78,6 +78,20 @@
 int contrad_conv2d_tile_order(const contrad_conv_desc* d, int mode, unsigned char* out, int capacity);
 int contrad_conv2d_wgrad(const contrad_conv_desc* d, const float* x, const float* gy, float* dwp,
                          float* dbias, float* workspace, long long workspace_bytes, contrad_stream_t stream);
+
+int contrad_conv2d_fwd_masked(const contrad_conv_desc* d, const float* x, const float* wp, const float* bias, float* y,
+                              float slope, float gain, float* workspace, long long workspace_bytes, const int* dead,
+                              int n_dead, contrad_stream_t stream);
+int contrad_conv2d_wgrad_masked(const contrad_conv_desc* d, const float* x, const float* gy, float* dwp, float* dbias,
+                                float* workspace, long long workspace_bytes, const int* dead, int n_dead,
+                                contrad_stream_t stream);
+int contrad_conv2d_dgrad_masked(const contrad_conv_desc* d, const float* gy, const float* wp, float* dx,
+                                const float* act_ref, float slope, float gain, float* workspace,
+                                long long workspace_bytes, const int* dead, int n_dead, contrad_stream_t stream);
+int contrad_conv2d_path_masked(const contrad_conv_desc* d, int mode, const int* dead, int n_dead);
+double contrad_conv2d_executed_fraction_masked(const contrad_conv_desc* d, int mode, const int* dead, int n_dead);
+long long contrad_conv2d_grid_blocks_masked(const contrad_conv_desc* d, int mode, int with_workspace, const int* dead,
+                                            int n_dead);
 
 long long contrad_contrast_workspace_bytes(int R, int D);
 int contrad_contrast_fwd(const float* z, int R, int D, int N, int mode, float inv_temp, float* lse,
```

Result: faster. 48360 images/sec, median of 6 (+1.4%).
